# yu45020/Text_Segmentation_Image_Inpainting

Hardware: NVIDIA H100
Metric: PartialConv UNet 512x512 images/sec (fwd+bwd) (higher is better)
Workload: dtype bf16

## Files before the change

text_segmentation_image_inpainting_b200/build.py:

```python
import fcntl
import hashlib
import os
import shutil
import subprocess
import sys

HERE = os.path.dirname(os.path.abspath(__file__))
CSRC = os.path.join(HERE, "csrc")
LIB = os.path.join(HERE, "libpconv_b200.so")
STAMP = os.path.join(HERE, "libpconv_b200.stamp")
SOURCES = ["api.cu", "conv_tc.cu", "conv_smallco.cu", "conv_k2r.cu", "conv_stem.cu", "conv_generic.cu", "elementwise.cu", "dwconv.cu", "seg_ops.cu", "inpaint_data.cu", "inpaint_loss.cu", "seg_data.cu", "seg_loss.cu"]
HEADERS = ["pcb_common.cuh", "pcb_ptx.cuh", "pil_data.cuh", os.path.join("..", "..", "include", "pconv_b200.h")]
NVCC_FLAGS = ["-gencode", "arch=compute_90a,code=sm_90a", "-O3", "-std=c++17", "-lineinfo",
              "-Xcompiler", "-fPIC", "-Xcompiler", "-fvisibility=hidden", "--expt-relaxed-constexpr",
              "-cudart", "static"]


def _nvcc():
    for cand in (os.environ.get("NVCC"), shutil.which("nvcc"), "/usr/local/cuda/bin/nvcc"):
        if cand and os.path.exists(cand):
            return cand
    raise RuntimeError("nvcc not found")


def _fingerprint(sources=None):
    h = hashlib.sha256()
    for d in [os.path.join(CSRC, s) for s in (SOURCES if sources is None else sources) + HEADERS] + [os.path.abspath(__file__)]:
        with open(d, "rb") as f:
            h.update(os.path.basename(d).encode() + b"\0" + f.read() + b"\0")
    h.update(" ".join(NVCC_FLAGS + os.environ.get("PCB_EXTRA_NVCC_FLAGS", "").split()).encode())
    return h.hexdigest()


def needs_build():
    if not os.path.exists(LIB):
        return True
    try:
        with open(STAMP) as f:
            return f.read().strip() != _fingerprint()
    except OSError:
        return True


def build(force=False, verbose=False):
    if not force and not needs_build():
        return LIB
    bdir = os.path.join(HERE, "build")
    os.makedirs(bdir, exist_ok=True)
    with open(os.path.join(bdir, ".lock"), "w") as lockf:
        fcntl.flock(lockf, fcntl.LOCK_EX)
        try:
            if not force and not needs_build():
                return LIB
            return _build_locked(bdir, verbose, force)
        finally:
            fcntl.flock(lockf, fcntl.LOCK_UN)


def _build_locked(bdir, verbose, force=False):
    nvcc = _nvcc()
    fp = _fingerprint()
    tag = f".{os.getpid()}.tmp"
    objs, procs = [], []
    stamps = {}
    for s in SOURCES:
        o = os.path.join(bdir, s.replace(".cu", ".o"))
        objs.append(o)
        stamps[o] = _fingerprint([s])
        try:
            if not force and os.path.exists(o) and open(o + ".stamp").read().strip() == stamps[o]:
                continue
        except OSError:
            pass
        cmd = [nvcc, *NVCC_FLAGS, *os.environ.get("PCB_EXTRA_NVCC_FLAGS", "").split(), "-c", os.path.join(CSRC, s), "-o", o + tag]
        if verbose:
            print(" ".join(cmd))
        procs.append((s, o, subprocess.Popen(cmd, stdout=subprocess.PIPE, stderr=subprocess.STDOUT)))
    failed = None
    for s, _o, p in procs:
        out, _ = p.communicate()
        if p.returncode and failed is None:
            failed = f"nvcc failed on {s}:\n{out.decode()}"
        if verbose and out:
            print(out.decode())
    if failed:
        for _s, o, _p in procs:
            if os.path.exists(o + tag):
                os.remove(o + tag)
        raise RuntimeError(failed)
    for _s, o, _p in procs:
        os.replace(o + tag, o)
        with open(o + ".stamp", "w") as f:
            f.write(stamps[o] + "\n")
    cmd = [nvcc, "-shared", "-o", LIB + tag, *objs, "-cudart", "static"]
    r = subprocess.run(cmd, stdout=subprocess.PIPE, stderr=subprocess.STDOUT)
    if r.returncode:
        raise RuntimeError("link failed:\n" + r.stdout.decode())
    os.replace(LIB + tag, LIB)
    with open(STAMP + tag, "w") as f:
        f.write(fp + "\n")
    os.replace(STAMP + tag, STAMP)
    return LIB


if __name__ == "__main__":
    print(build(force="--force" in sys.argv, verbose=True))
```

text_segmentation_image_inpainting_b200/csrc/conv_stem.cu:

```cuda
#include <string.h>

#include <algorithm>

#include "pcb_common.cuh"

namespace {

constexpr int S2D_C = 32;
constexpr int SK = 4;

size_t rup256(size_t v) { return (v + 255) / 256 * 256; }
size_t s2d_bytes(const pcb_conv *c) { return rup256(static_cast<size_t>(c->n) * (c->h / 2) * (c->w / 2) * S2D_C * sizeof(bf16)); }
size_t dwsub_bytes(const pcb_conv *c) { return rup256(sizeof(float) * c->cout * SK * SK * S2D_C); }

}

StemPlan pcb_stem_plan(const pcb_conv *c) {
    StemPlan K;
    memset(&K, 0, sizeof(K));
    if (c->dtype != PCB_BF16 || c->groups != 1 || c->nparts != 1 || c->kh != 7 || c->kw != 7 || c->stride != 2 || c->pad_h != 3 || c->pad_w != 3 ||
        c->dil != 1) return K;
    const pcb_part &p = c->parts[0];
    if (p.x_up || p.c > 8 || p.x_cstride != 8 || (p.mask && p.mask_up != 0) || ((c->h | c->w) & 1)) return K;
    if (p.x && (reinterpret_cast<uintptr_t>(p.x) & 15)) return K;
    if (c->ho != c->h / 2 || c->wo != c->w / 2 || c->cout < 32 || (c->cout & 7)) return K;
    pcb_conv &S = K.sub;
    S.n = c->n; S.h = c->h / 2; S.w = c->w / 2; S.cin = S2D_C; S.cout = c->cout; S.kh = S.kw = SK; S.stride = 1; S.pad_h = S.pad_w = 2; S.dil = 1;
    S.groups = 1; S.ho = S.h; S.wo = S.w; S.dtype = PCB_BF16; S.no_guard = c->no_guard; S.nparts = 1;
    S.parts[0].x = nullptr; S.parts[0].mask = nullptr; S.parts[0].c = S2D_C; S.parts[0].x_cstride = S2D_C;
    if (!pcb_tc_eligible(&S)) return K;
    size_t de;
    pcb_tc_weight_layout(&S, &K.sub_fe, &de);
    K.sub_fe = (K.sub_fe + 63) / 64 * 64;
    K.fwd_extra = K.sub_fe + 2 * static_cast<size_t>(c->cout) * SK * SK * S2D_C;
    K.workspace = s2d_bytes(c) + dwsub_bytes(c) + pcb_tc_workspace(&S);
    K.ok = true;
    return K;
}

namespace {

__global__ void s2d_kernel(const bf16 *__restrict__ x, const uint8_t *__restrict__ mask, bf16 *__restrict__ xs, int n, int h, int w) {
    const int hs = h >> 1, ws = w >> 1;
    const long long total = static_cast<long long>(n) * hs * ws * 2;
    for (long long i = blockIdx.x * static_cast<long long>(blockDim.x) + threadIdx.x; i < total; i += static_cast<long long>(gridDim.x) * blockDim.x) {
        const int a = static_cast<int>(i & 1);
        const long long cell = i >> 1;
        const int sx = static_cast<int>(cell % ws);
        const long long t = cell / ws;
        const int sy = static_cast<int>(t % hs), img = static_cast<int>(t / hs);
        const long long q = (static_cast<long long>(img) * h + 2 * sy + a) * w + 2 * sx;
        uint4 v0 = __ldg(reinterpret_cast<const uint4 *>(x + q * 8)), v1 = __ldg(reinterpret_cast<const uint4 *>(x + q * 8 + 8));
        if (mask) {
            if (mask[q] == 0) v0 = make_uint4(0u, 0u, 0u, 0u);
            if (mask[q + 1] == 0) v1 = make_uint4(0u, 0u, 0u, 0u);
        }
        uint4 *dst = reinterpret_cast<uint4 *>(xs + cell * S2D_C + a * 16);
        dst[0] = v0; dst[1] = v1;
    }
}

__global__ void stem_weight_kernel(const float *__restrict__ w, float *__restrict__ wsub, int cout, int cin) {
    const int i = blockIdx.x * blockDim.x + threadIdx.x;
    if (i >= cout * SK * SK * S2D_C) return;
    const int k = i % S2D_C, jb = (i / S2D_C) % SK, ja = (i / (S2D_C * SK)) % SK, co = i / (S2D_C * SK * SK);
    const int ch = k & 7, b = (k >> 3) & 1, a = k >> 4;
    const int ty = 2 * ja + a - 1, tx = 2 * jb + b - 1;
    wsub[i] = (ty >= 0 && ty < 7 && tx >= 0 && tx < 7 && ch < cin) ? w[((static_cast<long long>(co) * 7 + ty) * 7 + tx) * cin + ch] : 0.f;
}

__global__ void stem_dw_gather_kernel(const float *__restrict__ dwsub, float *__restrict__ dw, int cout, int cin) {
    const int i = blockIdx.x * blockDim.x + threadIdx.x;
    if (i >= cout * 49 * cin) return;
    const int ch = i % cin, tx = (i / cin) % 7, ty = (i / (cin * 7)) % 7, co = i / (cin * 49);
    const int ja = (ty + 1) >> 1, a = (ty + 1) & 1, jb = (tx + 1) >> 1, b = (tx + 1) & 1;
    dw[i] += dwsub[((static_cast<long long>(co) * SK + ja) * SK + jb) * S2D_C + (a * 2 + b) * 8 + ch];
}

int run_s2d(const pcb_conv *c, bf16 *xs, cudaStream_t st) {
    const pcb_part &p = c->parts[0];
    PCB_CHECK(p.x != nullptr, "space-to-depth stem: null x");
    const long long total = static_cast<long long>(c->n) * (c->h / 2) * (c->w / 2) * 2;
    const int grid = static_cast<int>(std::max<long long>(1, std::min<long long>((total + 255) / 256, 16ll * pcb_num_sms())));
    s2d_kernel<<<grid, 256, 0, st>>>(static_cast<const bf16 *>(p.x), p.mask, xs, c->n, c->h, c->w);
    PCB_LAUNCH_CHECK();
    return 0;
}

}

int pcb_stem_weight_prepare(const pcb_conv *c, const StemPlan &K, const float *w_master, void *w_fwd_extra, bool zero_padding, cudaStream_t st) {
    PCB_CHECK(K.ok && w_fwd_extra, "space-to-depth stem: weight prepare on a layer that does not take this path");
    float *wsub = reinterpret_cast<float *>(static_cast<bf16 *>(w_fwd_extra) + K.sub_fe);
    const int total = c->cout * SK * SK * S2D_C;
    stem_weight_kernel<<<(total + 255) / 256, 256, 0, st>>>(w_master, wsub, c->cout, c->cin);
    PCB_LAUNCH_CHECK();
    return pcb_tc_weight_prepare(&K.sub, wsub, w_fwd_extra, nullptr, zero_padding, st);
}

int pcb_stem_forward(const pcb_conv *c, const StemPlan &K, const void *w_fwd_extra, const float *bias, void *y, int y_cstride,
                     const float *msum, void *workspace, double *bn_sums, const pcb_ep *ep, cudaStream_t st) {
    PCB_CHECK(K.ok && workspace, "space-to-depth stem forward: wrong layer / no workspace");
    uint8_t *ws = static_cast<uint8_t *>(workspace);
    bf16 *xs = reinterpret_cast<bf16 *>(ws);
    if (int rc = run_s2d(c, xs, st)) return rc;
    pcb_conv sub = K.sub;
    sub.parts[0].x = xs;
    uint64_t *sub_ws = reinterpret_cast<uint64_t *>(ws + s2d_bytes(c) + dwsub_bytes(c));
    if (int rc = pcb_tc_forward_mask_pass(&sub, sub_ws, st)) return rc;
    return pcb_tc_forward_ws(&sub, w_fwd_extra, bias, y, y_cstride, msum, sub_ws, true, bn_sums, ep, st);
}

int pcb_stem_wgrad(const pcb_conv *c, const StemPlan &K, const void *dc, int dc_cstride, float *dw, void *workspace, bool zero_dw,
                   cudaStream_t st) {
    PCB_CHECK(K.ok && workspace, "space-to-depth stem wgrad: wrong layer / no workspace");
    if (zero_dw) PCB_CUDA(cudaMemsetAsync(dw, 0, sizeof(float) * c->cout * 49 * c->cin, st));
    uint8_t *ws = static_cast<uint8_t *>(workspace);
    bf16 *xs = reinterpret_cast<bf16 *>(ws);
    float *dwsub = reinterpret_cast<float *>(ws + s2d_bytes(c));
    void *sub_ws = ws + s2d_bytes(c) + dwsub_bytes(c);
    if (int rc = run_s2d(c, xs, st)) return rc;
    pcb_conv sub = K.sub;
    sub.parts[0].x = xs;
    if (int rc = pcb_tc_wgrad(&sub, dc, dc_cstride, dwsub, sub_ws, true, st)) return rc;
    const int total = c->cout * 49 * c->cin;
    stem_dw_gather_kernel<<<(total + 255) / 256, 256, 0, st>>>(dwsub, dw, c->cout, c->cin);
    PCB_LAUNCH_CHECK();
    return 0;
}
```

text_segmentation_image_inpainting_b200/csrc/conv_tc.cu:

```cuda
#include <cuda.h>
#include <stdlib.h>
#include <string.h>

#include <algorithm>

#include "pcb_common.cuh"
#include "pcb_ptx.cuh"

namespace {

constexpr int BLOCK_M = 128;
constexpr int BLOCK_K = 64;
constexpr int A_STAGE_BYTES = BLOCK_M * 128;
constexpr int NUM_PRODUCER_THREADS = 128;
constexpr int TC_MAX_PARTS = 2;
constexpr int MMA_WARPS = 8;
constexpr int MMA_THREADS = MMA_WARPS * 32;
constexpr int acc_pitch(int block_n) { return block_n + 4; }
constexpr int acc_stage_bytes(int block_n) { return BLOCK_M * acc_pitch(block_n) * 4; }

inline int rup(int v, int m) { return (v + m - 1) / m * m; }

struct TcPart {
    const bf16 *x;
    const uint64_t *tapmask;
    const uint8_t *mask;
    bf16 *dx;
    int c, c8, kext, koff, choff, cstride, xup, mup, dx_cstride;
};

struct TcParams {
    int n, h, w, cin, cout, kh, kw, stride, pad_h, pad_w, dil, ho, wo;
    int m_total;
    int nparts, no_guard, rowpack;
    int ncols;
    int ring_a, ring_b;
    int ktap;
    TcPart parts[TC_MAX_PARTS];
    const float *bias; const float *msum; bf16 *y; int y_cstride;
    const bf16 *dc; int dc_cstride, dc_c8, dc_kext;
    const bf16 *relu_x; int relu_cstride;
    int *abort_flag;
    int box_w, box_h, box_n, stages, use_fix;
    int wk_base, wk_row, wk_col;
    int sub, py, px, fh, fw;
    double *bn_sums;
    int bn_c;
    const float *ep_scale, *ep_shift;
    int ep_on, ep_act;
    float ep_slope;
};

constexpr int STAT_SLICE = 256;
constexpr int STAT_SMEM_BYTES = MMA_WARPS * STAT_SLICE * 4 + 16;
constexpr int EPI_WARPS = 4;
constexpr int EPI_STAT_SLICE = 512;
constexpr int EPI_STAT_SQ = EPI_STAT_SLICE / 2;
constexpr int EPI_STAT_SMEM_BYTES = EPI_WARPS * EPI_STAT_SLICE * 4;
constexpr int bf16_pitch(int block_n) { return block_n + 8; }
constexpr int bf16_stage_bytes(int block_n) { return BLOCK_M * bf16_pitch(block_n) * 2; }

__device__ __forceinline__ float warp_transpose_sum16(float (&v)[16], int lane) {
#pragma unroll
    for (int i = 0; i < 16; ++i) v[i] += __shfl_xor_sync(0xffffffffu, v[i], 16);
#pragma unroll
    for (int off = 8, n = 16; off >= 1; off >>= 1, n >>= 1) {
        const bool upper = (lane & off) != 0;
#pragma unroll
        for (int i = 0; i < 8; ++i) {
            if (i < (n >> 1)) {
                const float send = upper ? v[i] : v[i + (n >> 1)];
                const float keep = upper ? v[i + (n >> 1)] : v[i];
                v[i] = keep + __shfl_xor_sync(0xffffffffu, send, off);
            }
        }
    }
    return v[0];
}

__device__ __forceinline__ float warp_transpose_sum(float (&v)[32], int lane) {
#pragma unroll
    for (int off = 16, n = 32; off >= 1; off >>= 1, n >>= 1) {
        const bool upper = (lane & off) != 0;
#pragma unroll
        for (int i = 0; i < 16; ++i) {
            if (i < (n >> 1)) {
                const float send = upper ? v[i] : v[i + (n >> 1)];
                const float keep = upper ? v[i + (n >> 1)] : v[i];
                v[i] = keep + __shfl_xor_sync(0xffffffffu, send, off);
            }
        }
    }
    return v[0];
}

__device__ __forceinline__ uint32_t align1024(uint32_t a) { return (a + 1023u) & ~1023u; }

__device__ __forceinline__ void load_acc32(const float *src, uint32_t (&r)[32]) {
#pragma unroll
    for (int j = 0; j < 8; ++j) {
        const uint4 v = reinterpret_cast<const uint4 *>(src)[j];
        r[4 * j] = v.x; r[4 * j + 1] = v.y; r[4 * j + 2] = v.z; r[4 * j + 3] = v.w;
    }
}

struct EpiRow {
    long long mo;
    int m;
    bool rvalid, hole;
    float inv;
    float dscale[TC_MAX_PARTS];
};

template <int MODE>
__device__ __forceinline__ EpiRow tc_epi_row(const TcParams &P, int m, bool renorm = true) {
    EpiRow er;
    er.m = m;
    er.rvalid = m < P.m_total;
    er.inv = 0.f;
    er.hole = false;
    er.mo = m;
    int en = 0, eh = 0, ew = 0;
    if (MODE == 1 && er.rvalid) {
        en = m / (P.h * P.w); const int rem = m - en * P.h * P.w; eh = rem / P.w; ew = rem - eh * P.w;
        eh = eh * P.sub + P.py; ew = ew * P.sub + P.px;
        er.mo = (static_cast<long long>(en) * P.fh + eh) * P.fw + ew;
    }
    if (MODE == 0 && er.rvalid && renorm) {
        const float s = P.msum ? P.msum[er.mo] : 1.f;
        er.hole = (s == 0.f) && !P.no_guard;
        er.inv = er.hole ? 0.f : 1.0f / s;
    }
#pragma unroll
    for (int p = 0; p < TC_MAX_PARTS; ++p) {
        er.dscale[p] = 1.f;
        if (MODE == 1 && p < P.nparts) {
            const TcPart &pt = P.parts[p];
            if (er.rvalid && pt.dx != nullptr && pt.mask != nullptr)
                er.dscale[p] = pt.mask[(static_cast<long long>(en) * (P.fh >> pt.mup) + (eh >> pt.mup)) * (P.fw >> pt.mup) + (ew >> pt.mup)] ? 1.f : 0.f;
        }
    }
    return er;
}

template <int BLOCK_N, int MODE>
__device__ __forceinline__ void tc_epilogue(const TcParams &P, const EpiRow &er, const float *acc_row, int lane, int n0, float *s_stat,
                                            int cb, int ce, int sq_off) {
                const bool rvalid = er.rvalid, hole = er.hole;
                const long long mo = er.mo;
    #pragma unroll 1
                for (int c0 = cb; c0 < ce; c0 += 32) {
                    uint32_t r[32];
                    load_acc32(acc_row + c0, r);
                    const int col = n0 + c0;
                    bf16 *orow = nullptr;
                    int nstore = 0;
                    float scale = er.inv;
                    if (MODE == 0) {
                        if (rvalid && col < P.y_cstride) { orow = P.y + mo * P.y_cstride + col; nstore = min(32, P.y_cstride - col); }
                    } else {
                        scale = 1.f;
#pragma unroll
                        for (int p = 0; p < TC_MAX_PARTS; ++p) {
                            if (p >= P.nparts) break;
                            const TcPart &pt = P.parts[p];
                            const int local = col - pt.koff;
                            if (local >= 0 && local < pt.kext && pt.dx != nullptr && local < pt.c8 && rvalid) {
                                orow = pt.dx + mo * pt.dx_cstride + local;
                                nstore = min(32, pt.c8 - local);
                                scale = er.dscale[p];
                            }
                        }
                    }
                    const bool stats = (MODE == 0) && (s_stat != nullptr);
                    if (__any_sync(0xffffffffu, nstore > 0) || stats) {
                        uint4 o[4];
                        __nv_bfloat162 *ob = reinterpret_cast<__nv_bfloat162 *>(o);
                        float bl = 0.f;
                        const bool has_bias = (MODE == 0) && (P.bias != nullptr);
                        if (has_bias && col + lane < P.cout) bl = P.bias[col + lane];
                        const bool edge = (MODE == 0) && (col + 32 > P.cout);
                        const bool ep = (MODE == 0) && (P.ep_on != 0);
                        float el = 1.f, eh = 0.f;
                        if (ep && P.ep_scale != nullptr && col + lane < P.cout) { el = P.ep_scale[col + lane]; eh = P.ep_shift[col + lane]; }
    #pragma unroll
                        for (int j = 0; j < 16; ++j) {
                            float a = __uint_as_float(r[2 * j]), b = __uint_as_float(r[2 * j + 1]);
                            if (MODE == 0) {
                                const float b0 = has_bias ? __shfl_sync(0xffffffffu, bl, 2 * j) : 0.f;
                                const float b1 = has_bias ? __shfl_sync(0xffffffffu, bl, 2 * j + 1) : 0.f;
                                a = hole ? 0.f : fmaf(a, scale, b0);
                                b = hole ? 0.f : fmaf(b, scale, b1);
                                if (ep) {
                                    a = apply_act(fmaf(a, __shfl_sync(0xffffffffu, el, 2 * j), __shfl_sync(0xffffffffu, eh, 2 * j)), P.ep_act, P.ep_slope);
                                    b = apply_act(fmaf(b, __shfl_sync(0xffffffffu, el, 2 * j + 1), __shfl_sync(0xffffffffu, eh, 2 * j + 1)), P.ep_act, P.ep_slope);
                                }
                                if (edge) {
                                    if (col + 2 * j >= P.cout) a = 0.f;
                                    if (col + 2 * j + 1 >= P.cout) b = 0.f;
                                }
                            } else {
                                a *= scale; b *= scale;
                            }
                            ob[j] = __floats2bfloat162_rn(a, b);
                        }
                        if (nstore > 0) {
                            uint4 *dst = reinterpret_cast<uint4 *>(orow);
    #pragma unroll
                            for (int j = 0; j < 4; ++j)
                                if (j * 8 < nstore) dst[j] = o[j];
                        }
                        if (stats) {
                            float v[32], q[32];
                            const float live = rvalid ? 1.f : 0.f;
    #pragma unroll
                            for (int j = 0; j < 16; ++j) {
                                const float2 f = __bfloat1622float2(ob[j]);
                                v[2 * j] = f.x * live; v[2 * j + 1] = f.y * live;
                                q[2 * j] = v[2 * j] * v[2 * j]; q[2 * j + 1] = v[2 * j + 1] * v[2 * j + 1];
                            }
                            const float cs = warp_transpose_sum(v, lane), cq = warp_transpose_sum(q, lane);
                            s_stat[c0 - cb + lane] += cs;
                            s_stat[sq_off + c0 - cb + lane] += cq;
                        }
                    }
                }
}

template <int BLOCK_N>
__device__ __forceinline__ void tc_stats_flush(const TcParams &P, float *s_stat, int lane, int n0, int cb, int ce, int sq_off) {
    __syncwarp();
    for (int c0 = cb; c0 < ce; c0 += 32) {
        const int co = n0 + c0 + lane;
        if (co < P.bn_c) {
            atomicAdd(P.bn_sums + co, static_cast<double>(s_stat[c0 - cb + lane]));
            atomicAdd(P.bn_sums + P.bn_c + co, static_cast<double>(s_stat[sq_off + c0 - cb + lane]));
        }
        s_stat[c0 - cb + lane] = 0.f; s_stat[sq_off + c0 - cb + lane] = 0.f;
    }
    __syncwarp();
}

template <int BLOCK_N>
struct EpiRole {
    static constexpr int HN = (BLOCK_N >= 64) ? BLOCK_N / 2 : BLOCK_N;
    int q, half, cb, ce;
    __device__ __forceinline__ explicit EpiRole(int e) {
        q = 2 * (e >> 2) + (e & 1);
        half = (e & 3) >> 1;
        cb = half * HN;
        ce = (cb + HN <= BLOCK_N) ? cb + HN : cb;
    }
    __device__ __forceinline__ int slice() const { return half * 4 + q; }
};

template <int BLOCK_N>
__device__ __forceinline__ void stage_acc(const float (&acc)[BLOCK_N / 2], float *stage, int e, int lane) {
    constexpr int PITCH = acc_pitch(BLOCK_N);
    const int r0 = 64 * (e >> 2) + 16 * (e & 3) + (lane >> 2), c0 = 2 * (lane & 3);
#pragma unroll
    for (int i = 0; i < BLOCK_N / 2; i += 2) {
        const int row = r0 + 8 * ((i >> 1) & 1), col = 8 * (i >> 2) + c0;
        *reinterpret_cast<float2 *>(stage + row * PITCH + col) = make_float2(acc[i], acc[i + 1]);
    }
}

template <int BLOCK_N, int MODE>
__device__ __forceinline__ void mma_epilogue(const TcParams &P, const float (&acc)[BLOCK_N / 2], float *stage, int e, int lane, int m0, int n0,
                                             float *s_stat) {
    constexpr int PITCH = acc_pitch(BLOCK_N);
    const int g = e >> 2;
    stage_acc<BLOCK_N>(acc, stage, e, lane);
    ptx::named_sync(1 + g, 128);
    const EpiRole<BLOCK_N> R(e);
    const EpiRow er = tc_epi_row<MODE>(P, m0 + R.q * 32 + lane);
    tc_epilogue<BLOCK_N, MODE>(P, er, stage + (R.q * 32 + lane) * PITCH, lane, n0, s_stat, R.cb, R.ce, 128);
    ptx::named_sync(1 + g, 128);
}

template <int BLOCK_N>
__device__ __forceinline__ void tc_stats_final(const TcParams &P, const float *stat_base, int w, int lane, int stat_n0) {
    for (int col = w * 32 + lane; col < BLOCK_N; col += EPI_WARPS * 32) {
        const int co = stat_n0 + col;
        if (co < P.bn_c) {
            float a = 0.f, q = 0.f;
#pragma unroll
            for (int w4 = 0; w4 < EPI_WARPS; ++w4) { a += stat_base[w4 * EPI_STAT_SLICE + col]; q += stat_base[w4 * EPI_STAT_SLICE + EPI_STAT_SQ + col]; }
            atomicAdd(P.bn_sums + co, static_cast<double>(a));
            atomicAdd(P.bn_sums + P.bn_c + co, static_cast<double>(q));
        }
    }
}

template <int R> __device__ __forceinline__ void zero_acc(float (&a)[R]) {
#pragma unroll
    for (int i = 0; i < R; ++i) a[i] = 0.f;
}

constexpr int PERSIST_THREADS = 4 * 32 + MMA_THREADS + 32;
constexpr int MAX_RING = 8;

template <int BLOCK_N, int MODE>
__global__ void __launch_bounds__(PERSIST_THREADS, 1)
pconv_tc_persistent_kernel(const __grid_constant__ TcParams P, const __grid_constant__ CUtensorMap tmap_w) {
    constexpr int B_STAGE_BYTES = BLOCK_N * 128;
    extern __shared__ uint8_t smem_raw[];
    const uint32_t smem_base = align1024(ptx::smem_u32(smem_raw));
    const int SA = P.ring_a, SB = P.ring_b;
    const uint32_t sB = smem_base;
    const uint32_t sA = sB + SB * B_STAGE_BYTES;
    const uint32_t sBar = (sA + SA * A_STAGE_BYTES + 15u) & ~15u;
    const uint32_t bar_full_a = sBar, bar_empty_a = sBar + 8 * MAX_RING;
    const uint32_t bar_full_b = sBar + 16 * MAX_RING, bar_empty_b = sBar + 24 * MAX_RING;
    const uint32_t s_stat_addr = sBar + 32 * MAX_RING;
    const uint32_t s_acc = (s_stat_addr + STAT_SMEM_BYTES + 15u) & ~15u;
    float *acc_stage = reinterpret_cast<float *>(smem_raw + (s_acc - ptx::smem_u32(smem_raw)));

    const int warp = threadIdx.x >> 5, lane = threadIdx.x & 31;
    const int taps = P.kh * P.kw;
    const int np = (MODE == 0) ? P.nparts : 1;
    const int n_tiles = P.ncols / BLOCK_N;
    const int num_tiles = ((P.m_total + BLOCK_M - 1) / BLOCK_M) * n_tiles;

    auto tile_active = [&](int n0) -> bool {
        if (MODE == 0) return true;
        for (int p = 0; p < P.nparts; ++p)
            if (P.parts[p].dx && n0 < P.parts[p].koff + P.parts[p].kext && n0 + BLOCK_N > P.parts[p].koff) return true;
        return false;
    };

    if (threadIdx.x == 0) {
        for (int s = 0; s < MAX_RING; ++s) {
            ptx::mbar_init(bar_full_a + 8 * s, NUM_PRODUCER_THREADS); ptx::mbar_init(bar_empty_a + 8 * s, 2);
            ptx::mbar_init(bar_full_b + 8 * s, 1); ptx::mbar_init(bar_empty_b + 8 * s, 2);
        }
        ptx::fence_mbar_init();
    }
    if (warp == 12 && lane == 0) ptx::prefetch_tmap(&tmap_w);
    __syncthreads();

    if (warp < 4) {
        const int t = threadIdx.x;
        const int chunk = t & 7, r0 = t >> 3;
        const int plane = (MODE == 0) ? P.ho * P.wo : P.h * P.w;
        const int pwid = (MODE == 0) ? P.wo : P.w;
        int it = 0;
        bool dead = false;
        uint64_t wnext[TC_MAX_PARTS][8];
        auto issue_mask_loads = [&](int tl) {
#pragma unroll
            for (int p = 0; p < TC_MAX_PARTS; ++p)
#pragma unroll
                for (int i = 0; i < 8; ++i) wnext[p][i] = 0ull;
            if (MODE != 0 || tl >= num_tiles) return;
            const int tm0 = (tl / n_tiles) * BLOCK_M;
#pragma unroll
            for (int i = 0; i < 8; ++i) {
                const int idx = tm0 + r0 + 16 * i;
                if (idx >= P.m_total) continue;
#pragma unroll
                for (int p = 0; p < TC_MAX_PARTS; ++p)
                    if (p < P.nparts) wnext[p][i] = __ldg(P.parts[p].tapmask + idx);
            }
        };
        issue_mask_loads(blockIdx.x);
        for (int tile = blockIdx.x; tile < num_tiles && !dead; tile += gridDim.x) {
            const int m0 = (tile / n_tiles) * BLOCK_M, n0 = (tile % n_tiles) * BLOCK_N;
            uint64_t wcur[TC_MAX_PARTS][8];
#pragma unroll
            for (int p = 0; p < TC_MAX_PARTS; ++p)
#pragma unroll
                for (int i = 0; i < 8; ++i) wcur[p][i] = wnext[p][i];
            issue_mask_loads(tile + gridDim.x);
            if (!tile_active(n0)) continue;
            const uint32_t sw = static_cast<uint32_t>((chunk ^ (r0 & 7)) << 4);
            int ph[8], pw[8];
            int ibase[TC_MAX_PARTS][8];
            bool prow[8];
            const int ls = 31 - __clz(P.stride);
#pragma unroll
            for (int i = 0; i < 8; ++i) {
                const int m = m0 + r0 + 16 * i;
                prow[i] = m < P.m_total;
                const int mm = prow[i] ? m : 0;
                const int nn = mm / plane, rem = mm - nn * plane;
                const int hh = rem / pwid, ww = rem - hh * pwid;
                if (MODE == 0) {
                    ph[i] = hh * P.stride - P.pad_h; pw[i] = ww * P.stride - P.pad_w;
#pragma unroll
                    for (int p = 0; p < TC_MAX_PARTS; ++p)
                        ibase[p][i] = (p < P.nparts) ? nn * (P.h >> P.parts[p].xup) * (P.w >> P.parts[p].xup) * P.parts[p].cstride + chunk * 8 : 0;
                } else {
                    ph[i] = hh + P.pad_h; pw[i] = ww + P.pad_w;
                    ibase[0][i] = nn * P.ho * P.wo * P.dc_cstride + chunk * 8;
#pragma unroll
                    for (int p = 1; p < TC_MAX_PARTS; ++p) ibase[p][i] = 0;
                }
            }
            uint64_t tmv[TC_MAX_PARTS][8];
#pragma unroll
            for (int p = 0; p < TC_MAX_PARTS; ++p)
#pragma unroll
                for (int i = 0; i < 8; ++i) tmv[p][i] = wcur[p][i];

            auto push = [&](const bf16 *base, const int (&off)[8], const bool (&ok)[8]) -> bool {
                const int s = it % SA;
                if (!ptx::mbar_wait(bar_empty_a + 8 * s, ((it / SA) & 1) ^ 1, P.abort_flag, 101)) return false;
                const uint32_t dst = sA + s * A_STAGE_BYTES + r0 * 128 + sw;
#pragma unroll
                for (int i = 0; i < 8; ++i) ptx::cp_async_16(dst + i * (16 * 128), base + off[i], ok[i]);
                ptx::cp_async_mbar_arrive(bar_full_a + 8 * s);
                ptx::mbar_arrive(bar_full_a + 8 * s);
                ++it;
                return true;
            };
            if (MODE == 0 && P.rowpack) {
                const TcPart &pt = P.parts[0];
                const int cs = pt.cstride, rowpitch = P.w * cs;
                for (int tr = 0; tr < P.kh && !dead; ++tr) {
                    int off[8];
                    bool ok[8];
#pragma unroll
                    for (int i = 0; i < 8; ++i) {
                        const bool v = (chunk < P.kw) && ((tmv[0][i] >> (tr * P.kw + chunk)) & 1ull);
                        off[i] = v ? (ibase[0][i] - chunk * 8) + (ph[i] + tr * P.dil) * rowpitch + (pw[i] + chunk * P.dil) * cs : 0;
                        ok[i] = v;
                    }
                    if (!push(pt.x, off, ok)) dead = true;
                }
            } else {
                for (int tap = 0; tap < taps && !dead; ++tap) {
                    const int tr = tap / P.kw, tc = tap - tr * P.kw;
#pragma unroll
                    for (int p = 0; p < TC_MAX_PARTS; ++p) {
                        if (p >= np || dead) break;
                        const TcPart &pt = P.parts[p];
                        const bf16 *src = (MODE == 0) ? pt.x : P.dc;
                        const int cs = (MODE == 0) ? pt.cstride : P.dc_cstride;
                        const int xup = (MODE == 0) ? pt.xup : 0;
                        const int rowpitch = ((MODE == 0) ? (P.w >> xup) : P.wo) * cs;
                        int base[8];
                        bool rv[8];
#pragma unroll
                        for (int i = 0; i < 8; ++i) {
                            bool v;
                            int hi, wi;
                            if (MODE == 0) {
                                v = (tmv[p][i] >> tap) & 1ull;
                                hi = (ph[i] + tr * P.dil) >> xup; wi = (pw[i] + tc * P.dil) >> xup;
                            } else {
                                const int th = ph[i] - tr * P.dil, tw = pw[i] - tc * P.dil;
                                hi = th >> ls; wi = tw >> ls;
                                v = prow[i] && th >= 0 && tw >= 0 && ((th | tw) & (P.stride - 1)) == 0 && hi < P.ho && wi < P.wo;
                            }
                            base[i] = v ? ibase[p][i] + hi * rowpitch + wi * cs : 0;
                            rv[i] = v;
                        }
                        const int nb = ((MODE == 0) ? pt.kext : P.dc_kext) / BLOCK_K;
                        const int c8 = (MODE == 0) ? pt.c8 : P.dc_c8;
                        for (int cb = 0; cb < nb; ++cb) {
                            const bool cv = cb * BLOCK_K + chunk * 8 < c8;
                            int off[8];
                            bool ok[8];
#pragma unroll
                            for (int i = 0; i < 8; ++i) { ok[i] = rv[i] && cv; off[i] = ok[i] ? base[i] + cb * BLOCK_K : 0; }
                            if (!push(src, off, ok)) { dead = true; break; }
                        }
                    }
                }
            }
        }
        ptx::cp_async_wait<0>();
    } else if (warp == 12) {
        if (lane == 0) {
            int itb = 0;
            bool dead = false;
            auto load = [&](int kidx, int n0) -> bool {
                const int s = itb % SB;
                if (!ptx::mbar_wait(bar_empty_b + 8 * s, ((itb / SB) & 1) ^ 1, P.abort_flag, 103)) return false;
                ptx::mbar_arrive_expect_tx(bar_full_b + 8 * s, B_STAGE_BYTES);
                ptx::tma_load_2d(sB + s * B_STAGE_BYTES, &tmap_w, kidx, n0, bar_full_b + 8 * s);
                ++itb;
                return true;
            };
            for (int tile = blockIdx.x; tile < num_tiles && !dead; tile += gridDim.x) {
                const int n0 = (tile % n_tiles) * BLOCK_N;
                if (!tile_active(n0)) continue;
                const int num_kb = (MODE == 0) ? (P.rowpack ? P.kh : taps * (P.ktap / BLOCK_K)) : taps * (P.dc_kext / BLOCK_K);
                for (int kb = 0; kb < num_kb; ++kb)
                    if (!load(kb * BLOCK_K, n0)) { dead = true; break; }
            }
        }
    } else {
        const int e = warp - 4, g = e >> 2;
        const bool leader = (threadIdx.x & 127) == 0;
        const int num_a = (MODE == 0) ? (P.rowpack ? P.kh : taps * (P.ktap / BLOCK_K)) : taps * (P.dc_kext / BLOCK_K);
        const uint32_t a_rows = 64u * 128u;
        float *s_stat = (MODE == 0 && P.bn_sums != nullptr)
                            ? reinterpret_cast<float *>(smem_raw + (s_stat_addr - ptx::smem_u32(smem_raw))) : nullptr;
        const EpiRole<BLOCK_N> R(e);
        float *my_stat = s_stat ? s_stat + R.slice() * STAT_SLICE : nullptr;
        int stat_n0 = -1;
        if (my_stat) {
            for (int i = lane; i < STAT_SLICE; i += 32) my_stat[i] = 0.f;
            __syncwarp();
        }
        int ita = 0, itb = 0;
        bool dead = false;
        for (int tile = blockIdx.x; tile < num_tiles && !dead; tile += gridDim.x) {
            const int m0 = (tile / n_tiles) * BLOCK_M, n0 = (tile % n_tiles) * BLOCK_N;
            if (!tile_active(n0)) continue;
            if (my_stat && n0 != stat_n0) {
                if (stat_n0 >= 0) tc_stats_flush<BLOCK_N>(P, my_stat, lane, stat_n0, R.cb, R.ce, 128);
                stat_n0 = n0;
            }
            float acc[BLOCK_N / 2];
            zero_acc(acc);
            for (int a = 0; a < num_a && !dead; ++a, ++ita) {
                const int sa = ita % SA;
                if (!__all_sync(0xffffffffu, ptx::mbar_wait(bar_full_a + 8 * sa, (ita / SA) & 1, P.abort_flag, 104))) { dead = true; break; }
                ptx::fence_proxy_async_smem();
                const int sb = itb % SB;
                if (__all_sync(0xffffffffu, ptx::mbar_wait(bar_full_b + 8 * sb, (itb / SB) & 1, P.abort_flag, 105))) {
                    const uint64_t db = ptx::make_smem_desc(sB + sb * B_STAGE_BYTES, 16, 1024);
                    ptx::wgmma_fence();
                    const uint64_t da = ptx::make_smem_desc(sA + sa * A_STAGE_BYTES + g * a_rows, 16, 1024);
#pragma unroll
                    for (int k = 0; k < BLOCK_K / 16; ++k)
                        ptx::wgmma_bf16<BLOCK_N, 0, 0>(acc, da + 2 * k, db + 2 * k);
                    ptx::wgmma_commit();
                    ++itb;
                } else {
                    dead = true;
                }
                ptx::wgmma_wait<0>();
                ptx::wgmma_fence_regs(acc);
                if (leader) {
                    ptx::mbar_arrive(bar_empty_b + 8 * sb);
                    ptx::mbar_arrive(bar_empty_a + 8 * sa);
                }
            }
            if (dead) { stat_n0 = -1; break; }
            mma_epilogue<BLOCK_N, MODE>(P, acc, acc_stage, e, lane, m0, n0, my_stat);
        }
        if (my_stat && stat_n0 >= 0) tc_stats_flush<BLOCK_N>(P, my_stat, lane, stat_n0, R.cb, R.ce, 128);
    }
}


constexpr int EPI_WARP0 = MMA_WARPS + 4;
constexpr int TMA_THREADS = (EPI_WARP0 + EPI_WARPS) * 32;
constexpr int TMA_FIX_THREADS = 96;
constexpr int TMA_REGS = 128;
constexpr int TMA_CONSUMER_REGS = 192, TMA_SUPPORT_REGS = 64;
static_assert(TMA_THREADS == 512 && 2 * 128 * TMA_CONSUMER_REGS + 2 * 128 * TMA_SUPPORT_REGS == TMA_THREADS * TMA_REGS &&
              TMA_THREADS * TMA_REGS <= 65536, "TMA-fed fwd / dgrad register budget");

constexpr size_t TMA_BAR_BYTES = 24 * MAX_RING + 16;

template <int BLOCK_N, int MODE>
__device__ __forceinline__ void tc_epilogue_bf16(const TcParams &P, const EpiRow &er, const bf16 *srow, int lane, int n0, float *s_stat) {
    const bool stats = (MODE == 0) && (s_stat != nullptr);
#pragma unroll 1
    for (int c0 = 0; c0 < BLOCK_N; c0 += 32) {
        const int col = n0 + c0;
        bf16 *orow = nullptr;
        int nstore = 0;
        int xlocal = 0;
        float scale = 1.f;
        if (MODE == 0) {
            if (er.rvalid && col < P.y_cstride) { orow = P.y + er.mo * P.y_cstride + col; nstore = min(32, P.y_cstride - col); }
        } else {
#pragma unroll
            for (int p = 0; p < TC_MAX_PARTS; ++p) {
                if (p >= P.nparts) break;
                const TcPart &pt = P.parts[p];
                const int local = col - pt.koff;
                if (local >= 0 && local < pt.kext && pt.dx != nullptr && local < pt.c8 && er.rvalid) {
                    orow = pt.dx + er.mo * pt.dx_cstride + local;
                    nstore = min(32, pt.c8 - local);
                    scale = er.dscale[p];
                    xlocal = local;
                }
            }
        }
        if (nstore == 0 && !stats) continue;
        uint4 o[4];
#pragma unroll
        for (int j = 0; j < 4; ++j) o[j] = reinterpret_cast<const uint4 *>(srow + c0)[j];
        if (MODE == 1 && scale != 1.f) {
            __nv_bfloat162 *ob = reinterpret_cast<__nv_bfloat162 *>(o);
#pragma unroll
            for (int j = 0; j < 16; ++j) {
                const float2 f = __bfloat1622float2(ob[j]);
                ob[j] = __floats2bfloat162_rn(f.x * scale, f.y * scale);
            }
        }
        if (MODE == 1 && P.relu_x != nullptr && nstore > 0) {
            const uint4 *xr = reinterpret_cast<const uint4 *>(P.relu_x + er.mo * P.relu_cstride + xlocal);
#pragma unroll 1
            for (int j = 0; j < 4; ++j) {
                if (j * 8 >= nstore) break;
                const uint4 xv = xr[j];
                const __nv_bfloat162 *xb = reinterpret_cast<const __nv_bfloat162 *>(&xv);
                __nv_bfloat162 *ob = reinterpret_cast<__nv_bfloat162 *>(&o[j]);
#pragma unroll
                for (int k = 0; k < 4; ++k) {
                    const float2 xf = __bfloat1622float2(xb[k]);
                    const __nv_bfloat162 z = __float2bfloat162_rn(0.f);
                    ob[k] = __halves2bfloat162(xf.x <= 0.f ? z.x : ob[k].x, xf.y <= 0.f ? z.y : ob[k].y);
                }
            }
        }
        if (nstore > 0) {
            uint4 *dst = reinterpret_cast<uint4 *>(orow);
#pragma unroll
            for (int j = 0; j < 4; ++j)
                if (j * 8 < nstore) dst[j] = o[j];
        }
        if (stats) {
            const float live = er.rvalid ? 1.f : 0.f;
            const __nv_bfloat162 *ob = reinterpret_cast<const __nv_bfloat162 *>(srow + c0);
            float cs = 0.f, cq = 0.f;
#pragma unroll 1
            for (int h = 0; h < 2; ++h) {
                float v[16];
#pragma unroll
                for (int j = 0; j < 8; ++j) {
                    const float2 f = __bfloat1622float2(ob[8 * h + j]);
                    v[2 * j] = f.x * live; v[2 * j + 1] = f.y * live;
                }
                const float s = warp_transpose_sum16(v, lane);
#pragma unroll
                for (int j = 0; j < 8; ++j) {
                    const float2 f = __bfloat1622float2(ob[8 * h + j]);
                    const float a = f.x * live, b = f.y * live;
                    v[2 * j] = a * a; v[2 * j + 1] = b * b;
                }
                const float q = warp_transpose_sum16(v, lane);
                if ((lane >> 4) == h) { cs = s; cq = q; }
            }
            s_stat[c0 + lane] += cs;
            s_stat[EPI_STAT_SQ + c0 + lane] += cq;
        }
    }
}

template <int BLOCK_N, int MODE, typename TileFn>
__device__ __forceinline__ void tma_epilogue_warps(const TcParams &P, int tile0, int tstep, int num_tiles, TileFn tile_origin,
                                                   const bf16 *stage, uint32_t acc_full, uint32_t acc_empty, float *s_stat,
                                                   int &stat_n0, int w, int lane, int code) {
    const int row = w * 32 + lane;
    if (s_stat) {
        for (int i = lane; i < EPI_STAT_SLICE; i += 32) s_stat[i] = 0.f;
        __syncwarp();
    }
    uint32_t ph = 0;
    for (int tile = tile0; tile < num_tiles; tile += tstep) {
        int m0, n0;
        tile_origin(tile, m0, n0);
        if (n0 < 0) continue;
        if (s_stat && n0 != stat_n0) {
            if (stat_n0 >= 0) tc_stats_flush<BLOCK_N>(P, s_stat, lane, stat_n0, 0, BLOCK_N, EPI_STAT_SQ);
            stat_n0 = n0;
        }
        const EpiRow er = tc_epi_row<MODE>(P, m0 + row, false);
        if (!__all_sync(0xffffffffu, ptx::mbar_wait(acc_full, ph, P.abort_flag, code))) { stat_n0 = -1; return; }
        ph ^= 1;
        tc_epilogue_bf16<BLOCK_N, MODE>(P, er, stage + row * bf16_pitch(BLOCK_N), lane, n0, s_stat);
        __syncwarp();
        if (lane == 0) ptx::mbar_arrive(acc_empty);
    }
}

struct ConsRows {
    float inv[2];
    bool hole[2];
};
template <int MODE>
__device__ __forceinline__ ConsRows cons_rows(const TcParams &P, int m0, int e, int lane) {
    ConsRows cr;
#pragma unroll
    for (int h = 0; h < 2; ++h) {
        cr.inv[h] = 0.f; cr.hole[h] = false;
        if (MODE == 0) {
            const EpiRow er = tc_epi_row<0>(P, m0 + 64 * (e >> 2) + 16 * (e & 3) + (lane >> 2) + 8 * h);
            cr.inv[h] = er.inv; cr.hole[h] = er.hole;
        }
    }
    return cr;
}

template <int BLOCK_N, int MODE>
__device__ __forceinline__ void stage_acc_bf16(const TcParams &P, const float (&acc)[BLOCK_N / 2], bf16 *stage, int e, int lane, int n0,
                                               const ConsRows &cr) {
    constexpr int PITCH = bf16_pitch(BLOCK_N);
    const int r0 = 64 * (e >> 2) + 16 * (e & 3) + (lane >> 2), c0 = 2 * (lane & 3);
    const bool has_bias = (MODE == 0) && (P.bias != nullptr);
    const bool ep = (MODE == 0) && (P.ep_on != 0);
    const bool ep_aff = ep && (P.ep_scale != nullptr);
#pragma unroll
    for (int j = 0; j < BLOCK_N / 8; ++j) {
        const int col = n0 + 8 * j + c0;
        float b0 = 0.f, b1 = 0.f, s0 = 1.f, s1 = 1.f, t0 = 0.f, t1 = 0.f;
        if (MODE == 0) {
            const bool in0 = col < P.cout, in1 = col + 1 < P.cout;
            if (has_bias) { if (in0) b0 = __ldg(P.bias + col); if (in1) b1 = __ldg(P.bias + col + 1); }
            if (ep_aff) {
                if (in0) { s0 = __ldg(P.ep_scale + col); t0 = __ldg(P.ep_shift + col); }
                if (in1) { s1 = __ldg(P.ep_scale + col + 1); t1 = __ldg(P.ep_shift + col + 1); }
            }
        }
#pragma unroll
        for (int h = 0; h < 2; ++h) {
            float a = acc[4 * j + 2 * h], b = acc[4 * j + 2 * h + 1];
            if (MODE == 0) {
                a = cr.hole[h] ? 0.f : fmaf(a, cr.inv[h], b0);
                b = cr.hole[h] ? 0.f : fmaf(b, cr.inv[h], b1);
                if (ep) {
                    a = apply_act(fmaf(a, s0, t0), P.ep_act, P.ep_slope);
                    b = apply_act(fmaf(b, s1, t1), P.ep_act, P.ep_slope);
                }
                if (col >= P.cout) a = 0.f;
                if (col + 1 >= P.cout) b = 0.f;
            }
            *reinterpret_cast<__nv_bfloat162 *>(stage + (r0 + 8 * h) * PITCH + 8 * j + c0) = __floats2bfloat162_rn(a, b);
        }
    }
}

template <int BLOCK_N, int MODE>
__device__ __forceinline__ bool tma_stage_tile(const TcParams &P, const float (&acc)[BLOCK_N / 2], bf16 *stage, uint32_t acc_full,
                                               uint32_t acc_empty, uint32_t &ph, int e, int lane, int n0, const ConsRows &cr, int code) {
    if (!__all_sync(0xffffffffu, ptx::mbar_wait(acc_empty, ph, P.abort_flag, code))) return false;
    ph ^= 1;
    stage_acc_bf16<BLOCK_N, MODE>(P, acc, stage, e, lane, n0, cr);
    __syncwarp();
    if (lane == 0) ptx::mbar_arrive(acc_full);
    return true;
}

template <int BLOCK_N, int MODE, bool HALO>
__global__ void __maxnreg__(TMA_REGS)
pconv_tc_tma_kernel(const __grid_constant__ TcParams P, const __grid_constant__ CUtensorMap tmap_w,
                    const __grid_constant__ CUtensorMap tmap_a0, const __grid_constant__ CUtensorMap tmap_a1) {
    constexpr uint32_t B_BYTES = BLOCK_N * 128;
    extern __shared__ uint8_t smem_raw[];
    const uint32_t smem_base = align1024(ptx::smem_u32(smem_raw));
    const int S = P.stages;
    const int nB = HALO ? P.kw : 1;
    const int hx = HALO ? (P.kw - 1) * P.dil : 0;
    const uint32_t A_BYTES = static_cast<uint32_t>(BLOCK_M + hx) * 128u;
    const uint32_t A_ROOM = (A_BYTES + 1023u) & ~1023u;
    const uint32_t STAGE = A_ROOM + nB * B_BYTES;
    const uint32_t STAGE_TX = A_BYTES + nB * B_BYTES;
    const uint32_t sBar = smem_base + S * STAGE;
    const uint32_t bar_full = sBar, bar_fixed = sBar + 8 * MAX_RING, bar_empty = sBar + 16 * MAX_RING;
    const uint32_t acc_full = sBar + 24 * MAX_RING, acc_empty = acc_full + 8;
    const uint32_t s_stat_addr = sBar + TMA_BAR_BYTES;
    const uint32_t s_acc = s_stat_addr + EPI_STAT_SMEM_BYTES;
    uint8_t *smem_gen = smem_raw + (smem_base - ptx::smem_u32(smem_raw));

    const int warp = __shfl_sync(0xffffffffu, threadIdx.x >> 5, 0), lane = threadIdx.x & 31;
    const int np = (MODE == 0) ? P.nparts : 1;
    const int n_tiles = P.ncols / BLOCK_N;
    const int m_tiles = (P.m_total + BLOCK_M - 1) / BLOCK_M;
    const int num_tiles = m_tiles * n_tiles;
    const int tile0 = static_cast<int>(blockIdx.x), tstep = static_cast<int>(gridDim.x);
    auto m0_of = [&](int mt) -> int { return mt * BLOCK_M; };
    const bool fix = (MODE == 0) && P.use_fix;
    const int kwi = HALO ? 1 : P.kw;

    auto tile_active = [&](int n0) -> bool {
        if (MODE == 0) return true;
        for (int p = 0; p < P.nparts; ++p)
            if (P.parts[p].dx && n0 < P.parts[p].koff + P.parts[p].kext && n0 + BLOCK_N > P.parts[p].koff) return true;
        return false;
    };

    if (threadIdx.x == 0) {
        for (int s = 0; s < MAX_RING; ++s) {
            ptx::mbar_init(bar_full + 8 * s, 1); ptx::mbar_init(bar_fixed + 8 * s, TMA_FIX_THREADS / 32); ptx::mbar_init(bar_empty + 8 * s, 2);
        }
        ptx::mbar_init(acc_full, MMA_WARPS); ptx::mbar_init(acc_empty, EPI_WARPS);
        ptx::fence_mbar_init();
    }
    if (warp == 8 && lane == 0) { ptx::prefetch_tmap(&tmap_w); ptx::prefetch_tmap(&tmap_a0); if (np > 1) ptx::prefetch_tmap(&tmap_a1); }
    __syncthreads();

    float *s_stat = nullptr;
    int stat_n0 = -1;
    bf16 *acc_stage = reinterpret_cast<bf16 *>(smem_gen + (s_acc - smem_base));
    if (warp < MMA_WARPS) {
        ptx::setmaxnreg_inc<TMA_CONSUMER_REGS>();
        const int e = warp, g = warp >> 2;
        const bool leader = (threadIdx.x & 127) == 0;
        const uint32_t ready = fix ? bar_fixed : bar_full;
        const uint64_t desc_a0 = ptx::make_smem_desc(smem_base + g * 64 * 128, 16, 1024);
        const uint64_t desc_b0 = ptx::make_smem_desc(smem_base + A_ROOM, 16, 1024);
        const uint32_t stage16 = STAGE >> 4;
        const int shift0 = (HALO && MODE == 1) ? hx * 8 : 0;
        const int dshift = HALO ? ((MODE == 1) ? -P.dil * 8 : P.dil * 8) : 0;
        const int rows_a = P.kh * kwi;
        int nb0, nb1 = 0, kl0, kl1 = 4;
        {
            const int kext = (MODE == 0) ? P.parts[0].kext : P.dc_kext, c8 = (MODE == 0) ? P.parts[0].c8 : P.dc_c8;
            nb0 = kext / BLOCK_K; kl0 = min(4, (c8 - (nb0 - 1) * BLOCK_K + 15) >> 4);
            if (MODE == 0 && np > 1) { nb1 = P.parts[1].kext / BLOCK_K; kl1 = min(4, (P.parts[1].c8 - (nb1 - 1) * BLOCK_K + 15) >> 4); }
        }
        int s = 0;
        uint32_t ph = 0, aph = 1;
        bool dead = false;
        for (int tile = tile0; tile < num_tiles && !dead; tile += tstep) {
            const int n0 = (tile % n_tiles) * BLOCK_N;
            if (!tile_active(n0)) continue;
            const ConsRows cr = cons_rows<MODE>(P, m0_of(tile / n_tiles), e, lane);
            float acc[BLOCK_N / 2];
            zero_acc(acc);
            int held = -1;
            for (int r = 0; r < rows_a && !dead; ++r) {
#pragma unroll
                for (int p = 0; p < TC_MAX_PARTS; ++p) {
                    const int nbp = (p == 0) ? nb0 : nb1, klast = (p == 0) ? kl0 : kl1;
                    for (int cb = 0; cb < nbp; ++cb) {
                        if (!__all_sync(0xffffffffu, ptx::mbar_wait(ready + 8 * s, ph, P.abort_flag, 124))) { dead = true; break; }
                        uint64_t da = desc_a0 + static_cast<uint64_t>(s * stage16 + shift0), db = desc_b0 + static_cast<uint64_t>(s * stage16);
                        const int ksteps = (cb + 1 < nbp) ? 4 : klast;
                        ptx::wgmma_fence();
                        for (int tc = 0; tc < nB; ++tc, da += dshift, db += B_BYTES >> 4) {
                            if (ksteps == 4) {
#pragma unroll
                                for (int k = 0; k < 4; ++k) ptx::wgmma_bf16<BLOCK_N, 0, 0>(acc, da + 2 * k, db + 2 * k);
                            } else {
                                for (int k = 0; k < ksteps; ++k) ptx::wgmma_bf16<BLOCK_N, 0, 0>(acc, da + 2 * k, db + 2 * k);
                            }
                        }
                        ptx::wgmma_commit();
                        ptx::wgmma_wait<1>();
                        if (held >= 0 && leader) ptx::mbar_arrive(bar_empty + 8 * held);
                        held = s;
                        if (++s == S) { s = 0; ph ^= 1; }
                    }
                    if (dead) break;
                }
            }
            ptx::wgmma_wait<0>();
            ptx::wgmma_fence_regs(acc);
            if (held >= 0 && leader) ptx::mbar_arrive(bar_empty + 8 * held);
            if (dead) break;
            if (!tma_stage_tile<BLOCK_N, MODE>(P, acc, acc_stage, acc_full, acc_empty, aph, e, lane, n0, cr, 125)) break;
        }
    } else {
        ptx::setmaxnreg_dec<TMA_SUPPORT_REGS>();
        if (warp >= EPI_WARP0) {
            const int w = warp - EPI_WARP0;
            s_stat = (MODE == 0 && P.bn_sums != nullptr)
                         ? reinterpret_cast<float *>(smem_gen + (s_stat_addr - smem_base)) + w * EPI_STAT_SLICE : nullptr;
            auto origin = [&](int tile, int &m0, int &n0) {
                m0 = m0_of(tile / n_tiles); n0 = (tile % n_tiles) * BLOCK_N;
                if (!tile_active(n0)) n0 = -1;
            };
            tma_epilogue_warps<BLOCK_N, MODE>(P, tile0, tstep, num_tiles, origin, acc_stage, acc_full, acc_empty, s_stat, stat_n0, w, lane, 126);
            ptx::named_sync(1, EPI_WARPS * 32);
            if (s_stat != nullptr && stat_n0 >= 0) tc_stats_final<BLOCK_N>(P, s_stat - w * EPI_STAT_SLICE, w, lane, stat_n0);
        } else if (warp == 8) {
            int s = 0;
            uint32_t ph = 1;
            const int plane = (MODE == 0) ? P.ho * P.wo : P.h * P.w;
            const int pwid = (MODE == 0) ? P.wo : P.w;
            const int kext0 = (MODE == 0) ? P.parts[0].kext : P.dc_kext, kext1 = (MODE == 0 && np > 1) ? P.parts[1].kext : 0;
            const int dstep = (MODE == 0) ? P.dil : -P.dil;
            const int row_k = P.wk_row, col_k = P.wk_col;
            bool dead = false;
            for (int tile = tile0; tile < num_tiles && !dead; tile += tstep) {
                const int m0 = m0_of(tile / n_tiles), n0 = (tile % n_tiles) * BLOCK_N;
                if (!tile_active(n0)) continue;
                const int img = m0 / plane, rem = m0 - img * plane;
                const int oy = rem / pwid, ox = rem - oy * pwid;
                const int x_org = (MODE == 0) ? ox * P.stride - P.pad_w : (HALO ? ox + P.pad_w - hx : ox + P.pad_w);
                const int y_org = (MODE == 0) ? oy * P.stride - P.pad_h : oy + P.pad_h;
                int krow = P.wk_base;
                for (int tr = 0, y = y_org; tr < P.kh && !dead; ++tr, y += dstep, krow += row_k)
                    for (int ti = 0, x = x_org, kidx = krow; ti < kwi && !dead; ++ti, x += dstep, kidx = krow + ti * col_k) {
#pragma unroll
                        for (int p = 0; p < TC_MAX_PARTS; ++p) {
                            const int kext = (p == 0) ? kext0 : kext1;
                            const CUtensorMap *ma = (p == 0) ? &tmap_a0 : &tmap_a1;
                            for (int c0 = 0; c0 < kext; c0 += BLOCK_K, kidx += BLOCK_K) {
                                if (!__all_sync(0xffffffffu, ptx::mbar_wait(bar_empty + 8 * s, ph, P.abort_flag, 121))) { dead = true; break; }
                                if (ptx::elect_one()) {
                                    const uint32_t full = bar_full + 8 * s, dst = smem_base + s * STAGE;
                                    ptx::mbar_arrive_expect_tx(full, STAGE_TX);
                                    ptx::tma_load_4d(dst, ma, c0, x, y, img, full);
                                    uint32_t bdst = dst + A_ROOM;
                                    for (int tc = 0, kb = kidx; tc < nB; ++tc, kb += col_k, bdst += B_BYTES)
                                        ptx::tma_load_2d(bdst, &tmap_w, kb, n0, full);
                                }
                                __syncwarp();
                                if (++s == S) { s = 0; ph ^= 1; }
                            }
                            if (dead) break;
                        }
                    }
            }
        } else {
            if (fix) {
                constexpr int FR = HALO ? 3 : 2;
                const int t = (warp - 9) * 32 + lane;
                int s = 0;
                uint32_t ph = 0;
                bool dead = false;
                auto zero_row = [&](int row) {
                    uint4 *r = reinterpret_cast<uint4 *>(smem_gen + s * STAGE + row * 128);
                    const uint4 z = make_uint4(0u, 0u, 0u, 0u);
#pragma unroll
                    for (int k = 0; k < 8; ++k) r[k] = z;
                };
                if (!HALO) {
                    uint64_t wnext[FR][TC_MAX_PARTS];
                    auto load_words = [&](int tl) {
#pragma unroll
                        for (int r = 0; r < FR; ++r)
#pragma unroll
                            for (int p = 0; p < TC_MAX_PARTS; ++p) {
                                wnext[r][p] = 0ull;
                                const int m = m0_of(tl / n_tiles) + t + TMA_FIX_THREADS * r;
                                if (p < P.nparts && tl < num_tiles && t + TMA_FIX_THREADS * r < BLOCK_M && m < P.m_total)
                                    wnext[r][p] = __ldg(P.parts[p].tapmask + m);
                            }
                    };
                    load_words(tile0);
                    for (int tile = tile0; tile < num_tiles && !dead; tile += tstep) {
                        uint64_t wcur[FR][TC_MAX_PARTS];
#pragma unroll
                        for (int r = 0; r < FR; ++r)
#pragma unroll
                            for (int p = 0; p < TC_MAX_PARTS; ++p) wcur[r][p] = wnext[r][p];
                        load_words(tile + tstep);
                        if (MODE == 1 && !tile_active((tile % n_tiles) * BLOCK_N)) continue;
                        const int taps = P.kh * P.kw;
                        for (int tap = 0; tap < taps && !dead; ++tap) {
#pragma unroll
                            for (int p = 0; p < TC_MAX_PARTS; ++p) {
                                if (p >= np) break;
                                bool hole[FR], mine = false;
#pragma unroll
                                for (int r = 0; r < FR; ++r) {
                                    hole[r] = t + TMA_FIX_THREADS * r < BLOCK_M && ((wcur[r][p] >> tap) & 1ull) == 0ull;
                                    mine = mine || hole[r];
                                }
                                const bool any_hole = __any_sync(0xffffffffu, mine);
                                const int nb = ((MODE == 0) ? P.parts[p].kext : P.dc_kext) / BLOCK_K;
                                for (int cb = 0; cb < nb; ++cb) {
                                    if (!ptx::mbar_wait(bar_full + 8 * s, ph, P.abort_flag, 122)) { dead = true; break; }
                                    if (any_hole) {
#pragma unroll
                                        for (int r = 0; r < FR; ++r)
                                            if (hole[r]) zero_row(t + TMA_FIX_THREADS * r);
                                        ptx::fence_proxy_async_smem();
                                    }
                                    __syncwarp();
                                    if (lane == 0) ptx::mbar_arrive(bar_fixed + 8 * s);
                                    if (++s == S) { s = 0; ph ^= 1; }
                                }
                                if (dead) break;
                            }
                        }
                    }
                } else {
                    const int plane = P.ho * P.wo;
                    auto load_bits = [&](int tl, uint32_t (&b)[FR]) {
#pragma unroll
                        for (int r = 0; r < FR; ++r) b[r] = 0;
                        if (tl >= num_tiles) return;
                        const int m0 = m0_of(tl / n_tiles);
                        const int img = m0 / plane, rem = m0 - img * plane;
                        const int oy = rem / P.wo, ox = rem - oy * P.wo;
#pragma unroll
                        for (int p = 0; p < TC_MAX_PARTS; ++p) {
                            if (p >= P.nparts || P.parts[p].mask == nullptr) continue;
                            const int mup = P.parts[p].mup;
                            const uint8_t *mk = P.parts[p].mask + static_cast<long long>(img) * (P.h >> mup) * (P.w >> mup);
                            for (int tr = 0; tr < P.kh; ++tr) {
                                const int y = oy - P.pad_h + tr * P.dil;
                                if (y < 0 || y >= P.h) continue;
#pragma unroll
                                for (int r = 0; r < FR; ++r) {
                                    const int row = t + TMA_FIX_THREADS * r, x = ox - P.pad_w + row;
                                    if (row < BLOCK_M + hx && x >= 0 && x < P.w && __ldg(mk + (y >> mup) * (P.w >> mup) + (x >> mup)) == 0)
                                        b[r] |= 1u << (p * 8 + tr);
                                }
                            }
                        }
                    };
                    uint32_t nb_bits[FR];
                    load_bits(tile0, nb_bits);
                    for (int tile = tile0; tile < num_tiles && !dead; tile += tstep) {
                        uint32_t cb_bits[FR];
#pragma unroll
                        for (int r = 0; r < FR; ++r) cb_bits[r] = nb_bits[r];
                        load_bits(tile + tstep, nb_bits);
                        if (MODE == 1 && !tile_active((tile % n_tiles) * BLOCK_N)) continue;
                        for (int tr = 0; tr < P.kh && !dead; ++tr) {
#pragma unroll
                            for (int p = 0; p < TC_MAX_PARTS; ++p) {
                                if (p >= np) break;
                                bool hole[FR], mine = false;
#pragma unroll
                                for (int r = 0; r < FR; ++r) { hole[r] = (cb_bits[r] >> (p * 8 + tr)) & 1u; mine = mine || hole[r]; }
                                const bool any_hole = __any_sync(0xffffffffu, mine);
                                const int nb = ((MODE == 0) ? P.parts[p].kext : P.dc_kext) / BLOCK_K;
                                for (int cb = 0; cb < nb; ++cb) {
                                    if (!ptx::mbar_wait(bar_full + 8 * s, ph, P.abort_flag, 122)) { dead = true; break; }
                                    if (any_hole) {
#pragma unroll
                                        for (int r = 0; r < FR; ++r)
                                            if (hole[r]) zero_row(t + TMA_FIX_THREADS * r);
                                        ptx::fence_proxy_async_smem();
                                    }
                                    __syncwarp();
                                    if (lane == 0) ptx::mbar_arrive(bar_fixed + 8 * s);
                                    if (++s == S) { s = 0; ph ^= 1; }
                                }
                                if (dead) break;
                            }
                        }
                    }
                }
            }
        }
    }

}


constexpr int SP_MAX_ITEMS = 40;
struct SpItem { int dx, dy, wk; };
struct SpTable {
    int n_items;
    SpItem it[SP_MAX_ITEMS];
};

template <int BLOCK_N>
// ... 1264 lines not shown
    memset(ta, 0, sizeof(ta));
    for (int p = 0; p < c->nparts; ++p) {
        const pcb_part &pt = c->parts[p];
        const void *src = pt.x;
        long long cs = pt.x_cstride;
        const int c8 = rup(pt.c, 8);
        if (pt.x_up) {
            bf16 *up = reinterpret_cast<bf16 *>(static_cast<uint8_t *>(workspace) + T.up_off[p]);
            const long long pix = static_cast<long long>(c->n) * (c->h >> 1) * (c->w >> 1);
            const long long work = pix * (c8 >> 3);
            const int grid = static_cast<int>(std::min<long long>((work + 255) / 256, 16ll * pcb_num_sms()));
            upsample_part_kernel<<<grid, 256, 0, st>>>(static_cast<const bf16 *>(pt.x), pt.x_cstride, c8, pix, c->h >> 1, c->w >> 1, up);
            PCB_LAUNCH_CHECK();
            src = up; cs = c8;
        }
        if (pt.mask) *use_fix = 1;
        if (int rc = make_tmap_nhwc(&ta[p], src, c8, c->w, c->h, c->n, cs, bx, by, bn, c->stride)) return rc;
    }
    if (c->nparts < 2) ta[1] = ta[0];
    return 0;
}

pcb_smallco_layout smallco_layout(const Layout &L) {
    pcb_smallco_layout S;
    S.ktap = L.ktap; S.koff[0] = L.koff[0]; S.koff[1] = L.koff[1]; S.cout64 = L.cout64; S.kf = L.kf; S.kd = L.kd;
    return S;
}

}

bool pcb_tc_eligible(const pcb_conv *c) { return common_ok(c); }

size_t pcb_tc_workspace(const pcb_conv *c) { return tc_plan(c).workspace; }

void pcb_tc_weight_layout(const pcb_conv *c, size_t *fwd_elems, size_t *dgrad_elems) {
    const TcPlan T = tc_plan(c);
    *fwd_elems = T.fwd_elems;
    *dgrad_elems = T.dg_elems;
}

bool pcb_tc_subpixel(const pcb_conv *c) { return tc_plan(c).dg_at_source; }

void pcb_tc_routes(const pcb_conv *c, int32_t routes[3]) {
    static const int32_t code[] = {PCB_ROUTE_NONE, PCB_ROUTE_STEM, PCB_ROUTE_K2R, PCB_ROUTE_SMALLCO, PCB_ROUTE_TMA, PCB_ROUTE_TMA_S2,
                                   PCB_ROUTE_GATHER};
    const TcPlan T = tc_plan(c);
    routes[0] = code[T.fwd.route]; routes[1] = code[T.dg.route]; routes[2] = code[T.wg.route];
}

int pcb_tc_weight_prepare(const pcb_conv *c, const float *w_master, void *w_fwd, void *w_dgrad, bool zero_padding, cudaStream_t st) {
    const TcPlan T = tc_plan(c);
    const Layout &L = T.L;
    const size_t fe = T.fwd_elems, de = T.dg_elems;
    if (zero_padding) {
        PCB_CUDA(cudaMemsetAsync(w_fwd, 0, fe * 2, st));
        if (w_dgrad && de) PCB_CUDA(cudaMemsetAsync(w_dgrad, 0, de * 2, st));
    }
    WPrepParams W;
    memset(&W, 0, sizeof(W));
    W.cout = c->cout; W.taps = c->kh * c->kw; W.cin = c->cin; W.kw = c->kw; W.rowpack = L.rowpack; W.nparts = c->nparts;
    W.ktap = L.ktap; W.cout64 = L.cout64; W.kf = L.kf; W.kd = L.kd;
    int off = 0;
    for (int p = 0; p < c->nparts; ++p) { W.choff[p] = off; W.c[p] = c->parts[p].c; W.koff[p] = L.koff[p]; off += c->parts[p].c; }
    bf16 *wf = static_cast<bf16 *>(w_fwd), *wd = static_cast<bf16 *>(w_dgrad);
    if (!L.rowpack && W.taps <= 65535 && c->cout >= 32 && c->cin >= 32) {
        dim3 tg((c->cin + 31) / 32, (c->cout + 31) / 32, W.taps);
        tc_weight_prepare_tiled_kernel<<<tg, 256, 0, st>>>(w_master, W, wf, (w_dgrad && de) ? wd : nullptr);
    } else {
        const long long total = static_cast<long long>(c->cout) * W.taps * c->cin;
        const int grid = static_cast<int>(std::min<long long>((total + 1023) / 1024, 8ll * pcb_num_sms()));
        tc_weight_prepare_kernel<<<grid < 1 ? 1 : grid, 256, 0, st>>>(w_master, W, wf, (w_dgrad && de) ? wd : nullptr);
    }
    PCB_LAUNCH_CHECK();
    if (T.fwd.route == ROUTE_STEM) return pcb_stem_weight_prepare(c, T.stem, w_master, wf + T.extra_fwd_off, zero_padding, st);
    if (T.fwd.route == ROUTE_K2R) {
        PCB_CHECK(w_dgrad != nullptr, "kernel-to-row weights need the dgrad operand buffer");
        return pcb_k2r_weight_prepare(c, T.k2r, w_master, wf + T.extra_fwd_off, wd + T.extra_dg_off, zero_padding, st);
    }
    if (T.sp.ok) {
        PCB_CHECK(w_dgrad != nullptr, "sub-pixel weights need the dgrad operand buffer");
        return sp_weight_prepare(c, T.sp, L, w_master, wd + T.sp_off, st);
    }
    return 0;
}

int pcb_tc_forward_mask_pass(const pcb_conv *c, uint64_t *tapmask, cudaStream_t st) {
    const TcPlan T = tc_plan(c);
    PCB_CHECK(T.m_out < (1ll << 31), "problem too large");
    return T.fwd_tapmask ? launch_tapmask(c, tapmask, st) : 0;
}

bool pcb_tc_fuses_epilogue(const pcb_conv *c) { return tc_plan(c).fuses_epilogue; }

int pcb_tc_forward_ws(const pcb_conv *c, const void *w_fwd, const float *bias, void *y, int y_cstride, const float *msum,
                      uint64_t *tapmask, bool mask_pass_done, double *bn_sums, const pcb_ep *ep, cudaStream_t st) {
    int *flag = abort_flag_ptr();
    PCB_CHECK(flag != nullptr, "cudaMalloc(abort flag) failed");
    const TcPlan T = tc_plan(c);
    const Layout &L = T.L;
    const DirPlan &F = T.fwd;
    PCB_CHECK(T.m_out < (1ll << 31), "problem too large");
    PCB_CHECK(y_cstride % 8 == 0 && y_cstride >= c->cout, "tensor-core forward: y channel stride must be a multiple of 8 and >= cout");
    PCB_CHECK(bn_sums == nullptr || T.fuses_epilogue, "fused BatchNorm statistics requested from a kernel that does not produce them");
    PCB_CHECK(ep == nullptr || T.fuses_epilogue, "fused BatchNorm + activation requested from a kernel that does not apply it");
    if (!mask_pass_done && T.fwd_tapmask)
        if (int rc = launch_tapmask(c, tapmask, st)) return rc;
    const bf16 *wf = static_cast<const bf16 *>(w_fwd);
    if (F.route == ROUTE_STEM) return pcb_stem_forward(c, T.stem, wf + T.extra_fwd_off, bias, y, y_cstride, msum, tapmask, bn_sums, ep, st);
    if (F.route == ROUTE_K2R) return pcb_k2r_forward(c, T.k2r, smallco_layout(L), w_fwd, wf + T.extra_fwd_off, bias, y, y_cstride, msum, tapmask, st);
    if (F.route == ROUTE_SMALLCO) return pcb_smallco_forward(c, smallco_layout(L), w_fwd, bias, y, y_cstride, msum, st);
    TcParams P;
    base_params(P, c, L);
    P.m_total = static_cast<int>(T.m_out);
    fill_parts(c, L, P.parts, tapmask, T.m_out);
    P.bias = bias; P.msum = msum; P.y = static_cast<bf16 *>(y); P.y_cstride = y_cstride; P.abort_flag = flag;
    P.bn_sums = bn_sums; P.bn_c = c->cout;
    set_ep(P, ep);
    P.ncols = L.rows_f;
    CUtensorMap tm;
    if (int rc = make_tmap_2d(&tm, w_fwd, L.rows_f, L.kf, L.kf, F.bn)) return rc;
    if (F.route == ROUTE_TMA) {
        P.box_w = F.box_w; P.box_h = F.box_h; P.box_n = F.box_n;
        CUtensorMap ta[TC_MAX_PARTS];
        if (int rc = a_operand_maps(c, T, tapmask, F.box_w + (F.halo ? (c->kw - 1) * c->dil : 0), F.box_h, F.box_n, ta, &P.use_fix, st)) return rc;
        P.ncols = (c->cout <= 32) ? 32 : L.rows_f;
        P.wk_base = 0; P.wk_col = L.ktap; P.wk_row = c->kw * L.ktap;
        return launch_tma<0>(P, tm, ta[0], ta[1], F.bn, F.halo, st);
    }
    return launch_tc<0>(P, tm, F.bn, st);
}

bool pcb_tc_dgrad_fuses_relu(const pcb_conv *c) { return tc_plan(c).dg_fuses_relu; }

int pcb_tc_dgrad(const pcb_conv *c, const void *dc, int dc_cstride, const void *w_dgrad, void *const *dx, const int *dx_cstride,
                 cudaStream_t st, const void *relu_x, int relu_cstride) {
    const TcPlan T = tc_plan(c);
    const Layout &L = T.L;
    const DirPlan &D = T.dg;
    PCB_CHECK(D.route != ROUTE_NONE, "data gradient of a row-packed (cin <= 8) tensor-core layer: set force_generic and pass KRSC weights");
    PCB_CHECK(w_dgrad != nullptr && (reinterpret_cast<uintptr_t>(dc) & 15) == 0, "pcb_pconv_backward_data: w_dgrad required / dc misaligned");
    PCB_CHECK(relu_x == nullptr || (T.dg_fuses_relu && relu_cstride % 8 == 0 && relu_cstride >= rup(c->cin, 8) &&
                                    (reinterpret_cast<uintptr_t>(relu_x) & 15) == 0),
              "tensor-core dgrad: the ReLU backward is fused only on the TMA-fed stride-1 kernel (16-byte aligned input, channel stride %% 8 == 0)");
    int *flag = abort_flag_ptr();
    PCB_CHECK(flag != nullptr, "cudaMalloc(abort flag) failed");
    PCB_CHECK(T.m_in < (1ll << 31), "problem too large");
    PCB_CHECK(dc_cstride % 8 == 0 && dc_cstride >= rup(c->cout, 8), "tensor-core dgrad: dc channel stride must be a multiple of 8");
    const bf16 *wd = static_cast<const bf16 *>(w_dgrad);
    if (D.route == ROUTE_K2R) return pcb_k2r_dgrad(c, T.k2r, smallco_layout(L), dc, dc_cstride, w_dgrad, wd + T.extra_dg_off, dx, dx_cstride, st);
    if (D.route == ROUTE_SMALLCO) return pcb_smallco_dgrad(c, smallco_layout(L), dc, dc_cstride, w_dgrad, dx, dx_cstride, st);
    const SpPlan &SPL = T.sp;
    void *dx_local[TC_MAX_PARTS] = {nullptr, nullptr};
    for (int p = 0; p < c->nparts && p < TC_MAX_PARTS; ++p) dx_local[p] = dx[p];
    if (SPL.ok) {
        if (dx[SPL.pu] != nullptr)
            if (int rc = sp_dgrad_up(c, SPL, L, dc, dc_cstride, wd + T.sp_off, dx[SPL.pu], dx_cstride[SPL.pu], flag, st)) return rc;
        dx_local[SPL.pu] = nullptr;
        if (SPL.ps < 0 || dx[SPL.ps] == nullptr) return 0;
    }
    dx = dx_local;
    TcParams P;
    base_params(P, c, L);
    P.m_total = static_cast<int>(T.m_in);
    fill_parts(c, L, P.parts, nullptr, 0);
    for (int p = 0; p < c->nparts; ++p) {
        P.parts[p].dx = static_cast<bf16 *>(dx[p]);
        P.parts[p].dx_cstride = dx_cstride[p];
        PCB_CHECK(!dx[p] || (dx_cstride[p] % 8 == 0 && dx_cstride[p] >= P.parts[p].c8 && (reinterpret_cast<uintptr_t>(dx[p]) & 15) == 0),
                  "tensor-core dgrad: dx[%d] must be 16-byte aligned with a channel stride that is a multiple of 8", p);
    }
    P.dc = static_cast<const bf16 *>(dc); P.dc_cstride = dc_cstride; P.dc_c8 = rup(c->cout, 8); P.dc_kext = L.cout64;
    P.relu_x = static_cast<const bf16 *>(relu_x); P.relu_cstride = relu_cstride;
    P.abort_flag = flag;
    P.ncols = L.ktap;
    CUtensorMap tm;
    if (int rc = make_tmap_2d(&tm, w_dgrad, rup(L.ktap, 128), L.kd, L.kd, D.bn)) return rc;
    if (D.route == ROUTE_TMA) {
        P.box_w = D.box_w; P.box_h = D.box_h; P.box_n = D.box_n;
        P.wk_base = 0; P.wk_col = L.cout64; P.wk_row = c->kw * L.cout64;
        CUtensorMap ta;
        if (int rc = make_tmap_nhwc(&ta, dc, P.dc_c8, c->wo, c->ho, c->n, dc_cstride, D.box_w + (D.halo ? (c->kw - 1) * c->dil : 0), D.box_h, D.box_n, 1)) return rc;
        return launch_tma<1>(P, tm, ta, ta, D.bn, D.halo, st);
    }
    if (D.route == ROUTE_TMA_S2) {
        const int hh = c->h / 2, hw = c->w / 2;
        P.box_w = D.box_w; P.box_h = D.box_h; P.box_n = D.box_n;
        const bool fork = T.cls_fork;
        ClassStreams *CS = nullptr;
        if (fork) {
            if (int rc = class_streams(&CS)) return rc;
            PCB_CUDA(cudaEventRecord(CS->ev_fork, st));
        }
        for (int cls = 0; cls < 4; ++cls) {
            TcParams Q = P;
            const int py = cls >> 1, px = cls & 1;
            const int tr0 = (py + c->pad_h) & 1, tc0 = (px + c->pad_w) & 1;
            Q.kh = (c->kh - tr0 + 1) / 2; Q.kw = class_kw(c, px);
            Q.pad_h = (py + c->pad_h - tr0) / 2; Q.pad_w = (px + c->pad_w - tc0) / 2;
            Q.h = hh; Q.w = hw; Q.stride = 1; Q.dil = 1;
            Q.m_total = static_cast<int>(static_cast<long long>(c->n) * hh * hw);
            Q.sub = 2; Q.py = py; Q.px = px; Q.fh = c->h; Q.fw = c->w;
            Q.wk_base = (tr0 * c->kw + tc0) * L.cout64; Q.wk_row = 2 * c->kw * L.cout64; Q.wk_col = 2 * L.cout64;
            const bool halo = T.cls_halo[cls];
            CUtensorMap ta;
            if (int rc = make_tmap_nhwc(&ta, dc, P.dc_c8, c->wo, c->ho, c->n, dc_cstride, Q.box_w + (halo ? Q.kw - 1 : 0), Q.box_h, Q.box_n, 1)) return rc;
            cudaStream_t cs = (fork && cls > 0) ? CS->aux[cls - 1] : st;
            if (fork && cls > 0) PCB_CUDA(cudaStreamWaitEvent(cs, CS->ev_fork, 0));
            if (int rc = launch_tma<1>(Q, tm, ta, ta, D.bn, halo, cs)) return rc;
            if (fork && cls > 0) {
                PCB_CUDA(cudaEventRecord(CS->ev_join[cls - 1], cs));
                PCB_CUDA(cudaStreamWaitEvent(st, CS->ev_join[cls - 1], 0));
            }
        }
        return 0;
    }
    return launch_tc<1>(P, tm, D.bn, st);
}


template <int BLOCK_N, int T, bool HALO>
int launch_wgrad_tma(WgParams &P, const CUtensorMap &tdc, const CUtensorMap &ta0, const CUtensorMap &ta1, cudaStream_t st) {
    const int rows_a = 64 + (HALO ? (P.kw - 1) * P.dil : 0);
    PCB_CHECK(rows_a <= (HALO ? 3 : 1) * WGRAD_FIX_THREADS, "TMA-fed wgrad: %d-row A blocks exceed the fixer warps", rows_a);
    const size_t a_blk = (static_cast<size_t>(rows_a) * 128 + 1023) / 1024 * 1024;
    const size_t stage = (HALO ? 1 : T) * 2 * a_blk + static_cast<size_t>(BLOCK_N) * 128;
    P.stages = static_cast<int>(std::min<size_t>(MAX_RING, RING_BUDGET / stage));
    PCB_CHECK(P.stages >= 2, "TMA-fed wgrad: stage of %zu bytes does not fit twice", stage);
    const size_t smem = 1024 + P.stages * stage + 24 * MAX_RING;
    auto kern = pconv_tc_wgrad_tma_kernel<BLOCK_N, T, HALO>;
    PCB_SMEM_OPT_IN(kern, MAX_SMEM);
    P.tap_groups = HALO ? P.kh : (P.kh * P.kw + T - 1) / T;
    P.ci_tiles = (P.ktap + 127) / 128;
    const int co_tiles = (P.cout + BLOCK_N - 1) / BLOCK_N;
    const int base_ctas = co_tiles * P.tap_groups * P.ci_tiles;
    const int total_kb = (P.m_total + 63) / 64;
    int splits = (2 * pcb_num_sms() + base_ctas - 1) / base_ctas;
    splits = std::max(1, std::min(splits, total_kb));
    splits = std::min(splits, 65535);
    P.kb_per_split = (total_kb + splits - 1) / splits;
    splits = (total_kb + P.kb_per_split - 1) / P.kb_per_split;
    dim3 grid(base_ctas, splits);
    kern<<<grid, WGRAD_TMA_THREADS, smem, st>>>(P, tdc, ta0, ta1);
    PCB_LAUNCH_CHECK();
    return 0;
}

template <int BLOCK_N, int T, int STAGES>
static int launch_wgrad(WgParams &P, const CUtensorMap &tm, int cout, cudaStream_t st) {
    constexpr size_t smem = 1024 + STAGES * (T * 16384 + BLOCK_N * 128) + 24 * STAGES;
    auto kern = pconv_tc_wgrad_kernel<BLOCK_N, T, STAGES>;
    PCB_SMEM_OPT_IN(kern, (int)smem);
    P.tap_groups = (P.ntaps + T - 1) / T;
    P.ci_tiles = (P.ktap + 127) / 128;
    const int co_tiles = (cout + BLOCK_N - 1) / BLOCK_N;
    const int base_ctas = co_tiles * P.tap_groups * P.ci_tiles;
    const int total_kb = (P.m_total + 63) / 64;
    int splits = (4 * pcb_num_sms() + base_ctas - 1) / base_ctas;
    splits = std::max(1, std::min(splits, total_kb));
    splits = std::min(splits, 65535);
    P.kb_per_split = (total_kb + splits - 1) / splits;
    splits = (total_kb + P.kb_per_split - 1) / P.kb_per_split;
    dim3 grid(base_ctas, splits);
    kern<<<grid, WGRAD_THREADS, smem, st>>>(P, tm);
    PCB_LAUNCH_CHECK();
    return 0;
}

int pcb_tc_wgrad(const pcb_conv *c, const void *dc, int dc_cstride, float *dw, void *workspace, bool zero_dw, cudaStream_t st) {
    int *flag = abort_flag_ptr();
    PCB_CHECK(flag != nullptr, "cudaMalloc(abort flag) failed");
    PCB_CHECK(workspace != nullptr, "pcb_tc_wgrad: workspace required");
    const TcPlan T = tc_plan(c);
    const Layout &L = T.L;
    const DirPlan &W = T.wg;
    PCB_CHECK(T.m_out < (1ll << 31), "problem too large");
    PCB_CHECK(dc_cstride % 8 == 0 && dc_cstride >= c->cout, "tensor-core wgrad: dc channel stride must be a multiple of 8");
    if (W.route == ROUTE_STEM) return pcb_stem_wgrad(c, T.stem, dc, dc_cstride, dw, workspace, zero_dw, st);
    if (W.route == ROUTE_K2R) return pcb_k2r_wgrad(c, T.k2r, dc, dc_cstride, dw, workspace, zero_dw, st);
    if (W.route == ROUTE_SMALLCO) return pcb_smallco_wgrad(c, smallco_layout(L), dc, dc_cstride, dw, zero_dw, st);
    uint64_t *tapmask = static_cast<uint64_t *>(workspace);
    if (T.wg_tapmask)
        if (int rc = launch_tapmask(c, tapmask, st)) return rc;
    const size_t dw_bytes = sizeof(float) * c->cout * c->kh * c->kw * c->cin;
    if (zero_dw) PCB_CUDA(cudaMemsetAsync(dw, 0, dw_bytes, st));
    WgParams P;
    memset(&P, 0, sizeof(P));
    P.n = c->n; P.h = c->h; P.w = c->w; P.cin = c->cin; P.cout = c->cout; P.kh = c->kh; P.kw = c->kw; P.stride = c->stride;
    P.pad_h = c->pad_h; P.pad_w = c->pad_w; P.dil = c->dil; P.ho = c->ho; P.wo = c->wo; P.m_total = static_cast<int>(T.m_out);
    P.nparts = c->nparts; P.rowpack = L.rowpack; P.ktap = L.ktap; P.ntaps = L.rowpack ? c->kh : c->kh * c->kw;
    fill_parts(c, L, P.parts, tapmask, T.m_out);
    P.dw = dw; P.abort_flag = flag;
    CUtensorMap tm;
    if (int rc = make_tmap_2d(&tm, dc, T.m_out, c->cout, dc_cstride, 64)) return rc;
    if (W.route == ROUTE_TMA) {
        P.box_w = W.box_w; P.box_h = W.box_h; P.box_n = W.box_n;
        CUtensorMap ta[TC_MAX_PARTS];
        if (int rc = a_operand_maps(c, T, workspace, W.box_w + (W.halo ? (c->kw - 1) * c->dil : 0), W.box_h, W.box_n, ta, &P.use_fix, st)) return rc;
        if (W.bn == 128) return W.halo ? launch_wgrad_tma<128, 3, true>(P, tm, ta[0], ta[1], st) : launch_wgrad_tma<128, 3, false>(P, tm, ta[0], ta[1], st);
        return W.halo ? launch_wgrad_tma<64, 3, true>(P, tm, ta[0], ta[1], st) : launch_wgrad_tma<64, 3, false>(P, tm, ta[0], ta[1], st);
    }
    return launch_wgrad<64, 3, 3>(P, tm, c->cout, st);
}

int pcb_tc_read_abort_flag(int *value) {
    int *flag = abort_flag_ptr();
    PCB_CHECK(flag != nullptr, "no abort flag");
    PCB_CUDA(cudaMemcpy(value, flag, sizeof(int), cudaMemcpyDeviceToHost));
    if (*value != 0) cudaMemset(flag, 0, sizeof(int));
    return 0;
}
```

text_segmentation_image_inpainting_b200/csrc/pcb_common.cuh:

```cuda
#pragma once
#include <cuda_bf16.h>
#include <cuda_runtime.h>
#include <stdint.h>
#include <stdio.h>

#include "../../include/pconv_b200.h"

int pcb_set_error(const char *fmt, ...);
void pcb_count_launch(int n = 1);

#define PCB_CHECK(cond, ...)                       \
    do {                                           \
        if (!(cond)) return pcb_set_error(__VA_ARGS__); \
    } while (0)

#define PCB_CUDA(expr)                                                                           \
    do {                                                                                         \
        cudaError_t _e = (expr);                                                                 \
        if (_e != cudaSuccess)                                                                   \
            return pcb_set_error("%s:%d: %s -> %s", __FILE__, __LINE__, #expr, cudaGetErrorString(_e)); \
    } while (0)

#define PCB_LAUNCH_CHECK()                                                                        \
    do {                                                                                         \
        cudaError_t _e = cudaGetLastError();                                                     \
        if (_e != cudaSuccess)                                                                   \
            return pcb_set_error("%s:%d: kernel launch -> %s", __FILE__, __LINE__, cudaGetErrorString(_e)); \
        pcb_count_launch();                                                                      \
    } while (0)

constexpr int PCB_MAX_DEVICES = 64;

static inline int pcb_cur_device() {
    int dev = 0;
    cudaGetDevice(&dev);
    return (dev >= 0 && dev < PCB_MAX_DEVICES) ? dev : 0;
}

static inline int pcb_num_sms() {
    static int sms[PCB_MAX_DEVICES] = {0};
    const int dev = pcb_cur_device();
    if (!sms[dev]) {
        int v = 0;
        cudaDeviceGetAttribute(&v, cudaDevAttrMultiProcessorCount, dev);
        sms[dev] = v > 0 ? v : 132;
    }
    return sms[dev];
}

#define PCB_SMEM_OPT_IN(kern, bytes)                                                                          \
    do {                                                                                                      \
        static bool pcb_done_[PCB_MAX_DEVICES] = {};                                                          \
        const int pcb_dev_ = pcb_cur_device();                                                                \
        if (!pcb_done_[pcb_dev_]) {                                                                           \
            PCB_CUDA(cudaFuncSetAttribute(kern, cudaFuncAttributeMaxDynamicSharedMemorySize, (int)(bytes))); \
            pcb_done_[pcb_dev_] = true;                                                                       \
        }                                                                                                     \
    } while (0)

static inline size_t pcb_dtype_size(int dtype) { return dtype == PCB_BF16 ? 2 : 4; }

typedef __nv_bfloat16 bf16;

template <typename T> __device__ __forceinline__ float to_f32(T v);
template <> __device__ __forceinline__ float to_f32<float>(float v) { return v; }
template <> __device__ __forceinline__ float to_f32<bf16>(bf16 v) { return __bfloat162float(v); }

template <typename T> __device__ __forceinline__ T from_f32(float v);
template <> __device__ __forceinline__ float from_f32<float>(float v) { return v; }
template <> __device__ __forceinline__ bf16 from_f32<bf16>(float v) { return __float2bfloat16_rn(v); }

constexpr float PCB_SIGMOID_HALF_THRESHOLD = 8.940696716308594e-08f;
__device__ __forceinline__ bool sigmoid_above_half(float x) { return x > PCB_SIGMOID_HALF_THRESHOLD; }

__device__ __forceinline__ float apply_act(float z, int act, float slope) {
    if (act == PCB_ACT_RELU) return z > 0.f ? z : 0.f;
    if (act == PCB_ACT_LEAKY) return z > 0.f ? z : z * slope;
    if (act == PCB_ACT_RELU6) return fminf(fmaxf(z, 0.f), 6.f);
    return z;
}
__device__ __forceinline__ float act_grad(float z, int act, float slope) {
    if (act == PCB_ACT_RELU) return z > 0.f ? 1.f : 0.f;
    if (act == PCB_ACT_LEAKY) return z > 0.f ? 1.f : slope;
    if (act == PCB_ACT_RELU6) return (z > 0.f && z < 6.f) ? 1.f : 0.f;
    return 1.f;
}

template <typename T> struct Vec8;
template <> struct Vec8<bf16> {
    static __device__ __forceinline__ void load(const bf16 *p, float (&v)[8]) {
        uint4 r = *reinterpret_cast<const uint4 *>(p);
        const __nv_bfloat162 *h = reinterpret_cast<const __nv_bfloat162 *>(&r);
#pragma unroll
        for (int i = 0; i < 4; ++i) {
            float2 f = __bfloat1622float2(h[i]);
            v[2 * i] = f.x;
            v[2 * i + 1] = f.y;
        }
    }
    static __device__ __forceinline__ void store(bf16 *p, const float (&v)[8]) {
        uint4 r;
        __nv_bfloat162 *h = reinterpret_cast<__nv_bfloat162 *>(&r);
#pragma unroll
        for (int i = 0; i < 4; ++i) h[i] = __floats2bfloat162_rn(v[2 * i], v[2 * i + 1]);
        *reinterpret_cast<uint4 *>(p) = r;
    }
};
template <> struct Vec8<float> {
    static __device__ __forceinline__ void load(const float *p, float (&v)[8]) {
        float4 a = reinterpret_cast<const float4 *>(p)[0], b = reinterpret_cast<const float4 *>(p)[1];
        v[0] = a.x; v[1] = a.y; v[2] = a.z; v[3] = a.w; v[4] = b.x; v[5] = b.y; v[6] = b.z; v[7] = b.w;
    }
    static __device__ __forceinline__ void store(float *p, const float (&v)[8]) {
        reinterpret_cast<float4 *>(p)[0] = make_float4(v[0], v[1], v[2], v[3]);
        reinterpret_cast<float4 *>(p)[1] = make_float4(v[4], v[5], v[6], v[7]);
    }
};

__device__ __forceinline__ float warp_sum(float v) {
#pragma unroll
    for (int o = 16; o > 0; o >>= 1) v += __shfl_xor_sync(0xffffffffu, v, o);
    return v;
}

struct pcb_ep { const float *scale, *shift; int act; float slope; };

int pcb_generic_forward(const pcb_conv *c, const void *w, const float *bias, void *y, int y_cstride, const float *msum, cudaStream_t st);
int pcb_generic_dgrad(const pcb_conv *c, const void *dc, int dc_cstride, const void *w_krsc, void *const *dx, const int *dx_cstride,
                      cudaStream_t st);
int pcb_generic_wgrad(const pcb_conv *c, const void *dc, int dc_cstride, float *dw, bool zero_dw, cudaStream_t st);
int pcb_mask_sums(const pcb_conv *c, float *msum, uint8_t *newmask, cudaStream_t st);
bool pcb_tc_eligible(const pcb_conv *c);
size_t pcb_tc_workspace(const pcb_conv *c);
void pcb_tc_weight_layout(const pcb_conv *c, size_t *fwd_elems, size_t *dgrad_elems);
int pcb_tc_weight_prepare(const pcb_conv *c, const float *w_master, void *w_fwd, void *w_dgrad, bool zero_padding, cudaStream_t st);
int pcb_tc_forward_mask_pass(const pcb_conv *c, uint64_t *tapmask, cudaStream_t st);
int pcb_tc_forward_ws(const pcb_conv *c, const void *w_fwd, const float *bias, void *y, int y_cstride, const float *msum,
                      uint64_t *tapmask, bool mask_pass_done, double *bn_sums, const pcb_ep *ep, cudaStream_t st);
bool pcb_tc_fuses_epilogue(const pcb_conv *c);
bool pcb_tc_subpixel(const pcb_conv *c);
int pcb_tc_dgrad(const pcb_conv *c, const void *dc, int dc_cstride, const void *w_dgrad, void *const *dx, const int *dx_cstride,
                 cudaStream_t st, const void *relu_x = nullptr, int relu_cstride = 0);
bool pcb_tc_dgrad_fuses_relu(const pcb_conv *c);
int pcb_tc_wgrad(const pcb_conv *c, const void *dc, int dc_cstride, float *dw, void *workspace, bool zero_dw, cudaStream_t st);
int pcb_tc_read_abort_flag(int *value);
void pcb_tc_routes(const pcb_conv *c, int32_t routes[3]);
struct pcb_smallco_layout { int ktap, koff[2], cout64; long long kf, kd; };
bool pcb_smallco_eligible(const pcb_conv *c);
int pcb_smallco_forward(const pcb_conv *c, const pcb_smallco_layout &L, const void *w_fwd, const float *bias, void *y, int y_cstride, const float *msum,
                        cudaStream_t st);
int pcb_smallco_dgrad(const pcb_conv *c, const pcb_smallco_layout &L, const void *dc, int dc_cstride, const void *w_dgrad, void *const *dx, const int *dx_cstride,
                      cudaStream_t st);
int pcb_smallco_wgrad(const pcb_conv *c, const pcb_smallco_layout &L, const void *dc, int dc_cstride, float *dw, bool zero_dw, cudaStream_t st);
struct K2rPlan {
    bool ok;
    int pu, ps;
    int cu, cs, choff_u, choff_s;
    pcb_conv sub;
    size_t sub_fe, sub_de;
    size_t fwd_extra, dg_extra;
    size_t workspace;
};
K2rPlan pcb_k2r_plan(const pcb_conv *c);
int pcb_k2r_weight_prepare(const pcb_conv *c, const K2rPlan &K, const float *w_master, void *w_fwd_extra, void *w_dg_extra, bool zero_padding,
                           cudaStream_t st);
int pcb_k2r_forward(const pcb_conv *c, const K2rPlan &K, const pcb_smallco_layout &L, const void *w_fwd, const void *w_fwd_extra, const float *bias,
                    void *y, int y_cstride, const float *msum, void *workspace, cudaStream_t st);
int pcb_k2r_dgrad(const pcb_conv *c, const K2rPlan &K, const pcb_smallco_layout &L, const void *dc, int dc_cstride, const void *w_dgrad,
                  const void *w_dg_extra, void *const *dx, const int *dx_cstride, cudaStream_t st);
int pcb_k2r_wgrad(const pcb_conv *c, const K2rPlan &K, const void *dc, int dc_cstride, float *dw, void *workspace, bool zero_dw, cudaStream_t st);
struct StemPlan {
    bool ok;
    pcb_conv sub;
    size_t sub_fe;
    size_t fwd_extra;
    size_t workspace;
};
StemPlan pcb_stem_plan(const pcb_conv *c);
int pcb_stem_weight_prepare(const pcb_conv *c, const StemPlan &K, const float *w_master, void *w_fwd_extra, bool zero_padding, cudaStream_t st);
int pcb_stem_forward(const pcb_conv *c, const StemPlan &K, const void *w_fwd_extra, const float *bias, void *y, int y_cstride,
                     const float *msum, void *workspace, double *bn_sums, const pcb_ep *ep, cudaStream_t st);
int pcb_stem_wgrad(const pcb_conv *c, const StemPlan &K, const void *dc, int dc_cstride, float *dw, void *workspace, bool zero_dw,
                   cudaStream_t st);
bool pcb_dw_eligible(const pcb_conv *c);
int pcb_dw_weight_prepare(const pcb_conv *c, const float *w_master, void *w_t, cudaStream_t st);
int pcb_dw_forward(const pcb_conv *c, const void *w_t, const float *bias, void *y, int y_cstride, const float *msum, double *bn_sums,
                   const pcb_ep *ep, cudaStream_t st);
int pcb_dw_dgrad(const pcb_conv *c, const void *dc, int dc_cstride, const void *w_t, void *dx, int dx_cstride, cudaStream_t st);
int pcb_dw_wgrad(const pcb_conv *c, const void *dc, int dc_cstride, float *dw, bool zero_dw, cudaStream_t st);
```

text_segmentation_image_inpainting_b200/csrc/pcb_ptx.cuh:

```cuda
#pragma once
#include <cuda.h>
#include <cuda_runtime.h>
#include <stdint.h>

namespace ptx {

__device__ __forceinline__ uint32_t smem_u32(const void *p) { return static_cast<uint32_t>(__cvta_generic_to_shared(p)); }

__device__ __forceinline__ bool elect_one() {
    uint32_t pred = 0;
    asm volatile(
        "{\n\t.reg .pred P;\n\telect.sync _|P, 0xffffffff;\n\tselp.b32 %0, 1, 0, P;\n\t}" : "=r"(pred));
    return pred != 0;
}

__device__ __forceinline__ void mbar_init(uint32_t bar, uint32_t count) {
    asm volatile("mbarrier.init.shared::cta.b64 [%0], %1;" ::"r"(bar), "r"(count) : "memory");
}
__device__ __forceinline__ void fence_mbar_init() { asm volatile("fence.mbarrier_init.release.cluster;" ::: "memory"); }
__device__ __forceinline__ void mbar_arrive(uint32_t bar) {
    asm volatile("mbarrier.arrive.shared::cta.b64 _, [%0];" ::"r"(bar) : "memory");
}
__device__ __forceinline__ void mbar_arrive_expect_tx(uint32_t bar, uint32_t bytes) {
    asm volatile("mbarrier.arrive.expect_tx.shared::cta.b64 _, [%0], %1;" ::"r"(bar), "r"(bytes) : "memory");
}
__device__ __forceinline__ bool mbar_try_wait(uint32_t bar, uint32_t parity) {
    uint32_t ok;
    asm volatile(
        "{\n\t.reg .pred P;\n\t"
        "mbarrier.try_wait.parity.shared::cta.b64 P, [%1], %2;\n\t"
        "selp.b32 %0, 1, 0, P;\n\t}"
        : "=r"(ok)
        : "r"(bar), "r"(parity)
        : "memory");
    return ok != 0;
}
__device__ __forceinline__ bool mbar_wait(uint32_t bar, uint32_t parity, int *abort_flag, int code) {
    if (mbar_try_wait(bar, parity)) return true;
    const long long t0 = clock64();
    for (uint32_t it = 1;; ++it) {
        if (mbar_try_wait(bar, parity)) return true;
        if ((it & 63) == 0) {
            if (*reinterpret_cast<volatile int *>(abort_flag) != 0) return false;
            if (clock64() - t0 > 4000000000ll) break;
        }
    }
    atomicCAS(abort_flag, 0, code);
    return false;
}
__device__ __forceinline__ void cp_async_mbar_arrive(uint32_t bar) {
    asm volatile("cp.async.mbarrier.arrive.shared::cta.b64 [%0];" ::"r"(bar) : "memory");
}

__device__ __forceinline__ void cp_async_16(uint32_t dst, const void *src, bool valid) {
    const uint32_t sz = valid ? 16u : 0u;
    asm volatile("cp.async.cg.shared.global [%0], [%1], 16, %2;" ::"r"(dst), "l"(src), "r"(sz) : "memory");
}
__device__ __forceinline__ void cp_async_commit() { asm volatile("cp.async.commit_group;" ::: "memory"); }
template <int N> __device__ __forceinline__ void cp_async_wait() { asm volatile("cp.async.wait_group %0;" ::"n"(N) : "memory"); }

__device__ __forceinline__ void fence_proxy_async_smem() { asm volatile("fence.proxy.async.shared::cta;" ::: "memory"); }

__device__ __forceinline__ void prefetch_tmap(const CUtensorMap *m) {
    asm volatile("prefetch.tensormap [%0];" ::"l"(reinterpret_cast<uint64_t>(m)) : "memory");
}
__device__ __forceinline__ void tma_load_2d(uint32_t dst, const CUtensorMap *m, int c0, int c1, uint32_t bar) {
    asm volatile(
        "cp.async.bulk.tensor.2d.shared::cluster.global.mbarrier::complete_tx::bytes [%0], [%1, {%3, %4}], [%2];"
        ::"r"(dst), "l"(reinterpret_cast<uint64_t>(m)), "r"(bar), "r"(c0), "r"(c1)
        : "memory");
}
__device__ __forceinline__ void tma_load_4d(uint32_t dst, const CUtensorMap *m, int c0, int c1, int c2, int c3, uint32_t bar) {
    asm volatile(
        "cp.async.bulk.tensor.4d.shared::cluster.global.mbarrier::complete_tx::bytes [%0], [%1, {%3, %4, %5, %6}], [%2];"
        ::"r"(dst), "l"(reinterpret_cast<uint64_t>(m)), "r"(bar), "r"(c0), "r"(c1), "r"(c2), "r"(c3)
        : "memory");
}

__device__ __forceinline__ void wgmma_fence() { asm volatile("wgmma.fence.sync.aligned;" ::: "memory"); }
__device__ __forceinline__ void wgmma_commit() { asm volatile("wgmma.commit_group.sync.aligned;" ::: "memory"); }
template <int N> __device__ __forceinline__ void wgmma_wait() { asm volatile("wgmma.wait_group.sync.aligned %0;" ::"n"(N) : "memory"); }
template <int R> __device__ __forceinline__ void wgmma_fence_regs(float (&d)[R]) {
#pragma unroll
    for (int i = 0; i < R; ++i) asm volatile("" : "+f"(d[i])::"memory");
}
template <int TA, int TB> __device__ __forceinline__ void wgmma_m64n32(float (&d)[16], uint64_t a_desc, uint64_t b_desc) {
    asm volatile(
        "{\n\t"
        "wgmma.mma_async.sync.aligned.m64n32k16.f32.bf16.bf16 "
        "{%0, %1, %2, %3, %4, %5, %6, %7, %8, %9, %10, %11, %12, %13, %14, %15}, %16, %17, 1, 1, 1, %18, %19;\n\t"
        "}"
        : "+f"(d[0]), "+f"(d[1]), "+f"(d[2]), "+f"(d[3]), "+f"(d[4]), "+f"(d[5]), "+f"(d[6]), "+f"(d[7]), "+f"(d[8]), "+f"(d[9]), "+f"(d[10]), "+f"(d[11]), "+f"(d[12]), "+f"(d[13]), "+f"(d[14]), "+f"(d[15])
        : "l"(a_desc), "l"(b_desc), "n"(TA), "n"(TB));
}
template <int TA, int TB, int R> __device__ __forceinline__ void wgmma_m64n64(float (&d)[R], uint64_t a_desc, uint64_t b_desc) {
    static_assert(R >= 32, "m64n64 accumulator");
    asm volatile(
        "{\n\t"
        "wgmma.mma_async.sync.aligned.m64n64k16.f32.bf16.bf16 "
        "{%0, %1, %2, %3, %4, %5, %6, %7, %8, %9, %10, %11, %12, %13, %14, %15, %16, %17, %18, %19, %20, %21, %22, %23, %24, %25, %26, %27, %28, %29, %30, %31}, %32, %33, 1, 1, 1, %34, %35;\n\t"
        "}"
        : "+f"(d[0]), "+f"(d[1]), "+f"(d[2]), "+f"(d[3]), "+f"(d[4]), "+f"(d[5]), "+f"(d[6]), "+f"(d[7]), "+f"(d[8]), "+f"(d[9]), "+f"(d[10]), "+f"(d[11]), "+f"(d[12]), "+f"(d[13]), "+f"(d[14]), "+f"(d[15]), "+f"(d[16]), "+f"(d[17]), "+f"(d[18]), "+f"(d[19]), "+f"(d[20]), "+f"(d[21]), "+f"(d[22]), "+f"(d[23]), "+f"(d[24]), "+f"(d[25]), "+f"(d[26]), "+f"(d[27]), "+f"(d[28]), "+f"(d[29]), "+f"(d[30]), "+f"(d[31])
        : "l"(a_desc), "l"(b_desc), "n"(TA), "n"(TB));
}
template <int TA, int TB> __device__ __forceinline__ void wgmma_m64n128(float (&d)[64], uint64_t a_desc, uint64_t b_desc) {
    asm volatile(
        "{\n\t"
        "wgmma.mma_async.sync.aligned.m64n128k16.f32.bf16.bf16 "
        "{%0, %1, %2, %3, %4, %5, %6, %7, %8, %9, %10, %11, %12, %13, %14, %15, %16, %17, %18, %19, %20, %21, %22, %23, %24, %25, %26, %27, %28, %29, %30, %31, %32, %33, %34, %35, %36, %37, %38, %39, %40, %41, %42, %43, %44, %45, %46, %47, %48, %49, %50, %51, %52, %53, %54, %55, %56, %57, %58, %59, %60, %61, %62, %63}, %64, %65, 1, 1, 1, %66, %67;\n\t"
        "}"
        : "+f"(d[0]), "+f"(d[1]), "+f"(d[2]), "+f"(d[3]), "+f"(d[4]), "+f"(d[5]), "+f"(d[6]), "+f"(d[7]), "+f"(d[8]), "+f"(d[9]), "+f"(d[10]), "+f"(d[11]), "+f"(d[12]), "+f"(d[13]), "+f"(d[14]), "+f"(d[15]), "+f"(d[16]), "+f"(d[17]), "+f"(d[18]), "+f"(d[19]), "+f"(d[20]), "+f"(d[21]), "+f"(d[22]), "+f"(d[23]), "+f"(d[24]), "+f"(d[25]), "+f"(d[26]), "+f"(d[27]), "+f"(d[28]), "+f"(d[29]), "+f"(d[30]), "+f"(d[31]), "+f"(d[32]), "+f"(d[33]), "+f"(d[34]), "+f"(d[35]), "+f"(d[36]), "+f"(d[37]), "+f"(d[38]), "+f"(d[39]), "+f"(d[40]), "+f"(d[41]), "+f"(d[42]), "+f"(d[43]), "+f"(d[44]), "+f"(d[45]), "+f"(d[46]), "+f"(d[47]), "+f"(d[48]), "+f"(d[49]), "+f"(d[50]), "+f"(d[51]), "+f"(d[52]), "+f"(d[53]), "+f"(d[54]), "+f"(d[55]), "+f"(d[56]), "+f"(d[57]), "+f"(d[58]), "+f"(d[59]), "+f"(d[60]), "+f"(d[61]), "+f"(d[62]), "+f"(d[63])
        : "l"(a_desc), "l"(b_desc), "n"(TA), "n"(TB));
}
template <int N, int TA, int TB> __device__ __forceinline__ void wgmma_bf16(float (&d)[N / 2], uint64_t a_desc, uint64_t b_desc) {
    if constexpr (N == 32) wgmma_m64n32<TA, TB>(d, a_desc, b_desc);
    else if constexpr (N == 64) wgmma_m64n64<TA, TB>(d, a_desc, b_desc);
    else if constexpr (N == 128) wgmma_m64n128<TA, TB>(d, a_desc, b_desc);
    else {
        static_assert(N == 256 && TB == 0, "wgmma tile width");
        wgmma_m64n128<TA, TB>(*reinterpret_cast<float (*)[64]>(&d[0]), a_desc, b_desc);
        wgmma_m64n128<TA, TB>(*reinterpret_cast<float (*)[64]>(&d[64]), a_desc, b_desc + (16384 >> 4));
    }
}
template <int N> __device__ __forceinline__ void setmaxnreg_inc() { asm volatile("setmaxnreg.inc.sync.aligned.u32 %0;" ::"n"(N)); }
template <int N> __device__ __forceinline__ void setmaxnreg_dec() { asm volatile("setmaxnreg.dec.sync.aligned.u32 %0;" ::"n"(N)); }
__device__ __forceinline__ void named_sync(int id, int threads) { asm volatile("bar.sync %0, %1;" ::"r"(id), "r"(threads) : "memory"); }

__host__ __device__ __forceinline__ uint64_t make_smem_desc(uint32_t smem_addr, uint32_t lbo_bytes, uint32_t sbo_bytes) {
    uint64_t d = 0;
    d |= static_cast<uint64_t>((smem_addr >> 4) & 0x3FFFu);
    d |= static_cast<uint64_t>((lbo_bytes >> 4) & 0x3FFFu) << 16;
    d |= static_cast<uint64_t>((sbo_bytes >> 4) & 0x3FFFu) << 32;
    d |= 1ull << 62;
    return d;
}

}
```

Measured before the change: 1117.

## Replace stem space-to-depth sub-conv with dedicated warp-specialized wgmma fwd and wgrad kernels

The 7x7 stride-2 stem conv no longer goes through the generic tensor-core path on a space-to-depth tensor. It now uses its own forward kernel: the weights stay resident in shared memory, producer warps gather im2row chunks with cp.async, wgmma warps compute, and epilogue warps stage the output. A dedicated weight-gradient kernel is added too, and the space-to-depth channel count shrinks to 16 when the input has 4 or fewer channels, cutting padded work. This aims to remove generic-path overhead and wasted K, at the cost of a large amount of new, more complex and less general code.

```diff
diff --git a/text_segmentation_image_inpainting_b200/build.py b/text_segmentation_image_inpainting_b200/build.py
--- a/text_segmentation_image_inpainting_b200/build.py
+++ b/text_segmentation_image_inpainting_b200/build.py
@@ -10,7 +10,7 @@
 LIB = os.path.join(HERE, "libpconv_b200.so")
 STAMP = os.path.join(HERE, "libpconv_b200.stamp")
 SOURCES = ["api.cu", "conv_tc.cu", "conv_smallco.cu", "conv_k2r.cu", "conv_stem.cu", "conv_generic.cu", "elementwise.cu", "dwconv.cu", "seg_ops.cu", "inpaint_data.cu", "inpaint_loss.cu", "seg_data.cu", "seg_loss.cu"]
-HEADERS = ["pcb_common.cuh", "pcb_ptx.cuh", "pil_data.cuh", os.path.join("..", "..", "include", "pconv_b200.h")]
+HEADERS = ["pcb_common.cuh", "pcb_ptx.cuh", "pcb_tc_epi.cuh", "pil_data.cuh", os.path.join("..", "..", "include", "pconv_b200.h")]
 NVCC_FLAGS = ["-gencode", "arch=compute_90a,code=sm_90a", "-O3", "-std=c++17", "-lineinfo",
               "-Xcompiler", "-fPIC", "-Xcompiler", "-fvisibility=hidden", "--expt-relaxed-constexpr",
               "-cudart", "static"]
diff --git a/text_segmentation_image_inpainting_b200/csrc/conv_stem.cu b/text_segmentation_image_inpainting_b200/csrc/conv_stem.cu
--- a/text_segmentation_image_inpainting_b200/csrc/conv_stem.cu
+++ b/text_segmentation_image_inpainting_b200/csrc/conv_stem.cu
@@ -2,16 +2,16 @@
 
 #include <algorithm>
 
-#include "pcb_common.cuh"
+#include "pcb_tc_epi.cuh"
 
 namespace {
 
-constexpr int S2D_C = 32;
 constexpr int SK = 4;
 
 size_t rup256(size_t v) { return (v + 255) / 256 * 256; }
-size_t s2d_bytes(const pcb_conv *c) { return rup256(static_cast<size_t>(c->n) * (c->h / 2) * (c->w / 2) * S2D_C * sizeof(bf16)); }
-size_t dwsub_bytes(const pcb_conv *c) { return rup256(sizeof(float) * c->cout * SK * SK * S2D_C); }
+int rup64(int v) { return (v + 63) / 64 * 64; }
+size_t s2d_bytes(const pcb_conv *c, int sc) { return rup256(static_cast<size_t>(c->n) * (c->h / 2) * (c->w / 2) * sc * sizeof(bf16)); }
+size_t dwsub_bytes(const pcb_conv *c, int sc) { return rup256(sizeof(float) * c->cout * SK * SK * sc); }
 
 }
 
@@ -24,23 +24,19 @@
     if (p.x_up || p.c > 8 || p.x_cstride != 8 || (p.mask && p.mask_up != 0) || ((c->h | c->w) & 1)) return K;
     if (p.x && (reinterpret_cast<uintptr_t>(p.x) & 15)) return K;
     if (c->ho != c->h / 2 || c->wo != c->w / 2 || c->cout < 32 || (c->cout & 7)) return K;
-    pcb_conv &S = K.sub;
-    S.n = c->n; S.h = c->h / 2; S.w = c->w / 2; S.cin = S2D_C; S.cout = c->cout; S.kh = S.kw = SK; S.stride = 1; S.pad_h = S.pad_w = 2; S.dil = 1;
-    S.groups = 1; S.ho = S.h; S.wo = S.w; S.dtype = PCB_BF16; S.no_guard = c->no_guard; S.nparts = 1;
-    S.parts[0].x = nullptr; S.parts[0].mask = nullptr; S.parts[0].c = S2D_C; S.parts[0].x_cstride = S2D_C;
-    if (!pcb_tc_eligible(&S)) return K;
-    size_t de;
-    pcb_tc_weight_layout(&S, &K.sub_fe, &de);
-    K.sub_fe = (K.sub_fe + 63) / 64 * 64;
-    K.fwd_extra = K.sub_fe + 2 * static_cast<size_t>(c->cout) * SK * SK * S2D_C;
-    K.workspace = s2d_bytes(c) + dwsub_bytes(c) + pcb_tc_workspace(&S);
+    const long long lim = (1ll << 31) - 1, cells = static_cast<long long>(c->n) * c->ho * c->wo;
+    if (cells * rup64(c->cout) > lim || cells * 32 > lim) return K;
+    K.sc = p.c <= 4 ? 16 : 32;
+    const int bn_f = (c->cout % 128 == 0) ? 128 : 64;
+    K.fwd_extra = static_cast<size_t>((c->cout + bn_f - 1) / bn_f * bn_f) * SK * SK * 64 + 2 * static_cast<size_t>(c->cout) * SK * SK * 32;
+    K.workspace = s2d_bytes(c, 32) + dwsub_bytes(c, 32) + rup256(static_cast<size_t>(cells) * sizeof(uint64_t));
     K.ok = true;
     return K;
 }
 
 namespace {
 
-__global__ void s2d_kernel(const bf16 *__restrict__ x, const uint8_t *__restrict__ mask, bf16 *__restrict__ xs, int n, int h, int w) {
+__global__ void s2d_kernel(const bf16 *__restrict__ x, const uint8_t *__restrict__ mask, bf16 *__restrict__ xs, int n, int h, int w, int cc) {
     const int hs = h >> 1, ws = w >> 1;
     const long long total = static_cast<long long>(n) * hs * ws * 2;
     for (long long i = blockIdx.x * static_cast<long long>(blockDim.x) + threadIdx.x; i < total; i += static_cast<long long>(gridDim.x) * blockDim.x) {
@@ -50,81 +46,364 @@
         const long long t = cell / ws;
         const int sy = static_cast<int>(t % hs), img = static_cast<int>(t / hs);
         const long long q = (static_cast<long long>(img) * h + 2 * sy + a) * w + 2 * sx;
-        uint4 v0 = __ldg(reinterpret_cast<const uint4 *>(x + q * 8)), v1 = __ldg(reinterpret_cast<const uint4 *>(x + q * 8 + 8));
-        if (mask) {
-            if (mask[q] == 0) v0 = make_uint4(0u, 0u, 0u, 0u);
-            if (mask[q + 1] == 0) v1 = make_uint4(0u, 0u, 0u, 0u);
-        }
-        uint4 *dst = reinterpret_cast<uint4 *>(xs + cell * S2D_C + a * 16);
-        dst[0] = v0; dst[1] = v1;
-    }
-}
-
-__global__ void stem_weight_kernel(const float *__restrict__ w, float *__restrict__ wsub, int cout, int cin) {
+        const bool k0 = !mask || mask[q] != 0, k1 = !mask || mask[q + 1] != 0;
+        bf16 *dst = xs + cell * 4 * cc + a * 2 * cc;
+        if (cc == 4) {
+            const uint2 z = make_uint2(0u, 0u);
+            const uint2 v0 = k0 ? __ldg(reinterpret_cast<const uint2 *>(x + q * 8)) : z, v1 = k1 ? __ldg(reinterpret_cast<const uint2 *>(x + q * 8 + 8)) : z;
+            *reinterpret_cast<uint4 *>(dst) = make_uint4(v0.x, v0.y, v1.x, v1.y);
+        } else {
+            const uint4 z = make_uint4(0u, 0u, 0u, 0u);
+            reinterpret_cast<uint4 *>(dst)[0] = k0 ? __ldg(reinterpret_cast<const uint4 *>(x + q * 8)) : z;
+            reinterpret_cast<uint4 *>(dst)[1] = k1 ? __ldg(reinterpret_cast<const uint4 *>(x + q * 8 + 8)) : z;
+        }
+    }
+}
+
+struct StemK { int ja, jb, a, b, ch; };
+__host__ __device__ __forceinline__ StemK stem_k(int k, int sc) {
+    const int cc = sc >> 2;
+    StemK r;
+    r.ja = k / (4 * sc); r.jb = (k / sc) & 3; r.a = (k / (2 * cc)) & 1; r.b = (k / cc) & 1; r.ch = k % cc;
+    return r;
+}
+
+__global__ void stem_weight_kernel(const float *__restrict__ w, bf16 *__restrict__ wst, int cout, int rows, int cin, int sc) {
     const int i = blockIdx.x * blockDim.x + threadIdx.x;
-    if (i >= cout * SK * SK * S2D_C) return;
-    const int k = i % S2D_C, jb = (i / S2D_C) % SK, ja = (i / (S2D_C * SK)) % SK, co = i / (S2D_C * SK * SK);
-    const int ch = k & 7, b = (k >> 3) & 1, a = k >> 4;
-    const int ty = 2 * ja + a - 1, tx = 2 * jb + b - 1;
-    wsub[i] = (ty >= 0 && ty < 7 && tx >= 0 && tx < 7 && ch < cin) ? w[((static_cast<long long>(co) * 7 + ty) * 7 + tx) * cin + ch] : 0.f;
-}
-
-__global__ void stem_dw_gather_kernel(const float *__restrict__ dwsub, float *__restrict__ dw, int cout, int cin) {
+    if (i >= rows * SK * SK * sc) return;
+    const int co = i / (SK * SK * sc);
+    const StemK k = stem_k(i % (SK * SK * sc), sc);
+    const int ty = 2 * k.ja + k.a - 1, tx = 2 * k.jb + k.b - 1;
+    const bool in = co < cout && ty >= 0 && ty < 7 && tx >= 0 && tx < 7 && k.ch < cin;
+    wst[i] = __float2bfloat16_rn(in ? w[((static_cast<long long>(co) * 7 + ty) * 7 + tx) * cin + k.ch] : 0.f);
+}
+
+__global__ void stem_dw_gather_kernel(const float *__restrict__ dwsub, float *__restrict__ dw, int cout, int cin, int sc) {
     const int i = blockIdx.x * blockDim.x + threadIdx.x;
     if (i >= cout * 49 * cin) return;
     const int ch = i % cin, tx = (i / cin) % 7, ty = (i / (cin * 7)) % 7, co = i / (cin * 49);
     const int ja = (ty + 1) >> 1, a = (ty + 1) & 1, jb = (tx + 1) >> 1, b = (tx + 1) & 1;
-    dw[i] += dwsub[((static_cast<long long>(co) * SK + ja) * SK + jb) * S2D_C + (a * 2 + b) * 8 + ch];
-}
-
-int run_s2d(const pcb_conv *c, bf16 *xs, cudaStream_t st) {
+    dw[i] += dwsub[static_cast<long long>(co) * SK * SK * sc + (ja * SK + jb) * sc + (a * 2 + b) * (sc >> 2) + ch];
+}
+
+__device__ __forceinline__ void im2row_chunk(const bf16 *xs, int hs, int ws, int sc, bool rv, int img, int oy, int ox, int kidx, uint32_t dst) {
+    const int ja = kidx / (4 * sc), rem = kidx - ja * 4 * sc, jb = rem / sc, ch0 = rem - jb * sc;
+    const int y = oy + ja - 2, x = ox + jb - 2;
+    const bool ok = rv && y >= 0 && y < hs && x >= 0 && x < ws;
+    const bf16 *src = ok ? xs + ((static_cast<long long>(img) * hs + y) * ws + x) * sc + ch0 : xs;
+    ptx::cp_async_16_ca(dst, src, ok);
+}
+
+constexpr int STEM_THREADS = MMA_THREADS + 4 * 32 + EPI_WARPS * 32;
+constexpr int STEM_PROD_THREADS = 128;
+constexpr int STEM_EPI_WARP0 = MMA_WARPS + 4;
+constexpr uint32_t STEM_W_BLOCK = 64 * 128;
+
+struct StemFwdParams {
+    TcParams P;
+    const bf16 *xs, *wst;
+    int hs, ws, sc, nkb, n_tiles, stages;
+};
+
+__global__ void __launch_bounds__(STEM_THREADS, 1) stem_fwd_kernel(const __grid_constant__ StemFwdParams A) {
+    const TcParams &P = A.P;
+    extern __shared__ uint8_t smem_raw[];
+    const uint32_t smem_base = align1024(ptx::smem_u32(smem_raw));
+    uint8_t *smem_gen = smem_raw + (smem_base - ptx::smem_u32(smem_raw));
+    const int S = A.stages, nkb = A.nkb;
+    const uint32_t sW = smem_base, sA = sW + nkb * STEM_W_BLOCK;
+    const uint32_t sBar = sA + S * A_STAGE_BYTES;
+    const uint32_t bar_full = sBar, bar_empty = sBar + 8 * MAX_RING;
+    const uint32_t acc_full = sBar + 16 * MAX_RING, acc_empty = acc_full + 8;
+    const uint32_t s_stat_addr = sBar + TMA_BAR_BYTES;
+    bf16 *acc_stage = reinterpret_cast<bf16 *>(smem_gen + (s_stat_addr + EPI_STAT_SMEM_BYTES - smem_base));
+
+    const int warp = __shfl_sync(0xffffffffu, threadIdx.x >> 5, 0), lane = threadIdx.x & 31;
+    const int n0 = (blockIdx.x % A.n_tiles) * 64;
+    const int tile0 = blockIdx.x / A.n_tiles, tstep = gridDim.x / A.n_tiles;
+    const int m_tiles = (P.m_total + BLOCK_M - 1) / BLOCK_M;
+
+    if (threadIdx.x == 0) {
+        for (int s = 0; s < MAX_RING; ++s) { ptx::mbar_init(bar_full + 8 * s, STEM_PROD_THREADS); ptx::mbar_init(bar_empty + 8 * s, 2); }
+        ptx::mbar_init(acc_full, MMA_WARPS); ptx::mbar_init(acc_empty, EPI_WARPS);
+        ptx::fence_mbar_init();
+    }
+    const int kw = SK * SK * A.sc;
+    for (int i = threadIdx.x; i < nkb * 64 * 8; i += STEM_THREADS) {
+        const int kb = i >> 9, r = (i >> 3) & 63, ch = i & 7;
+        const uint4 v = __ldg(reinterpret_cast<const uint4 *>(A.wst + static_cast<long long>(n0 + r) * kw + kb * 64 + ch * 8));
+        *reinterpret_cast<uint4 *>(smem_gen + kb * STEM_W_BLOCK + r * 128 + ((ch ^ (r & 7)) << 4)) = v;
+    }
+    ptx::fence_proxy_async_smem();
+    __syncthreads();
+
+    if (warp < MMA_WARPS) {
+        const int e = warp, g = warp >> 2;
+        const bool leader = (threadIdx.x & 127) == 0;
+        const uint64_t desc_a0 = ptx::make_smem_desc(sA + g * 64 * 128, 16, 1024);
+        const uint64_t desc_w0 = ptx::make_smem_desc(sW, 16, 1024);
+        int s = 0;
+        uint32_t ph = 0, aph = 1;
+        bool dead = false;
+        for (int mt = tile0; mt < m_tiles && !dead; mt += tstep) {
+            const ConsRows cr = cons_rows<0>(P, mt * BLOCK_M, e, lane);
+            float acc[32];
+            zero_acc(acc);
+            int held = -1;
+            for (int kb = 0; kb < nkb; ++kb) {
+                if (!__all_sync(0xffffffffu, ptx::mbar_wait(bar_full + 8 * s, ph, P.abort_flag, 131))) { dead = true; break; }
+                ptx::fence_proxy_async_smem();
+                const uint64_t da = desc_a0 + static_cast<uint64_t>(s * (A_STAGE_BYTES >> 4));
+                const uint64_t dw = desc_w0 + static_cast<uint64_t>(kb * (STEM_W_BLOCK >> 4));
+                ptx::wgmma_fence();
+#pragma unroll
+                for (int k = 0; k < 4; ++k) ptx::wgmma_bf16<64, 0, 0>(acc, da + 2 * k, dw + 2 * k);
+                ptx::wgmma_commit();
+                ptx::wgmma_wait<1>();
+                if (held >= 0 && leader) ptx::mbar_arrive(bar_empty + 8 * held);
+                held = s;
+                if (++s == S) { s = 0; ph ^= 1; }
+            }
+            ptx::wgmma_wait<0>();
+            ptx::wgmma_fence_regs(acc);
+            if (held >= 0 && leader) ptx::mbar_arrive(bar_empty + 8 * held);
+            if (dead) break;
+            if (!tma_stage_tile<64, 0>(P, acc, acc_stage, acc_full, acc_empty, aph, e, lane, n0, cr, 132)) break;
+        }
+    } else if (warp < STEM_EPI_WARP0) {
+        const int t = threadIdx.x - MMA_THREADS, chunk = t & 7, r0 = t >> 3;
+        const uint32_t sw = static_cast<uint32_t>((chunk ^ (r0 & 7)) << 4);
+        const int plane = A.hs * A.ws;
+        int s = 0;
+        uint32_t ph = 1;
+        bool dead = false;
+        for (int mt = tile0; mt < m_tiles && !dead; mt += tstep) {
+            int img[8], oy[8], ox[8];
+            bool rv[8];
+#pragma unroll
+            for (int i = 0; i < 8; ++i) {
+                const int m = mt * BLOCK_M + r0 + 16 * i;
+                rv[i] = m < P.m_total;
+                const int mm = rv[i] ? m : 0;
+                img[i] = mm / plane;
+                const int rem = mm - img[i] * plane;
+                oy[i] = rem / A.ws; ox[i] = rem - oy[i] * A.ws;
+            }
+            for (int kb = 0; kb < nkb; ++kb) {
+                if (!ptx::mbar_wait(bar_empty + 8 * s, ph, P.abort_flag, 133)) { dead = true; break; }
+                const uint32_t dst = sA + s * A_STAGE_BYTES + r0 * 128 + sw;
+#pragma unroll
+                for (int i = 0; i < 8; ++i) im2row_chunk(A.xs, A.hs, A.ws, A.sc, rv[i], img[i], oy[i], ox[i], kb * 64 + chunk * 8, dst + i * 16 * 128);
+                ptx::cp_async_mbar_arrive(bar_full + 8 * s);
+                ptx::mbar_arrive(bar_full + 8 * s);
+                if (++s == S) { s = 0; ph ^= 1; }
+            }
+        }
+        ptx::cp_async_wait<0>();
+    } else {
+        const int w = warp - STEM_EPI_WARP0;
+        float *s_stat = P.bn_sums != nullptr ? reinterpret_cast<float *>(smem_gen + (s_stat_addr - smem_base)) + w * EPI_STAT_SLICE : nullptr;
+        int stat_n0 = -1;
+        auto origin = [&](int mt, int &m0, int &tn0) { m0 = mt * BLOCK_M; tn0 = n0; };
+        tma_epilogue_warps<64, 0>(P, tile0, tstep, m_tiles, origin, acc_stage, acc_full, acc_empty, s_stat, stat_n0, w, lane, 134);
+        ptx::named_sync(1, EPI_WARPS * 32);
+        if (s_stat != nullptr && stat_n0 >= 0) tc_stats_final<64>(P, s_stat - w * EPI_STAT_SLICE, w, lane, stat_n0);
+    }
+}
+
+constexpr int STEM_WG_THREADS = MMA_THREADS + 4 * 32;
+
+struct StemWgParams {
+    const bf16 *xs, *dc;
+    float *dwsub;
+    int *abort_flag;
+    int hs, ws, sc, cin, cout, dc_cstride, m_total, kb_per_cta, stages;
+};
+
+template <int MB>
+__global__ void __launch_bounds__(STEM_WG_THREADS, 1) stem_wgrad_kernel(const __grid_constant__ StemWgParams W) {
+    constexpr uint32_t BLK = 64 * 128;
+    constexpr uint32_t A_BYTES = 2 * MB * BLK, STAGE = A_BYTES + BLK;
+    extern __shared__ uint8_t smem_raw[];
+    const uint32_t smem_base = align1024(ptx::smem_u32(smem_raw));
+    const int S = W.stages;
+    const uint32_t bar_full = smem_base + S * STAGE, bar_empty = bar_full + 8 * MAX_RING;
+    const int warp = __shfl_sync(0xffffffffu, threadIdx.x >> 5, 0), lane = threadIdx.x & 31;
+    const int n0 = blockIdx.y * 64;
+    const int total_kb = (W.m_total + 63) / 64;
+    const int kb_begin = blockIdx.x * W.kb_per_cta;
+    const int num_kb = max(0, min(total_kb, kb_begin + W.kb_per_cta) - kb_begin);
+
+    if (threadIdx.x == 0) {
+        for (int s = 0; s < MAX_RING; ++s) { ptx::mbar_init(bar_full + 8 * s, STEM_PROD_THREADS); ptx::mbar_init(bar_empty + 8 * s, 2); }
+        ptx::fence_mbar_init();
+    }
+    __syncthreads();
+    if (warp < MMA_WARPS) {
+        const int g = warp >> 2;
+        const bool leader = (threadIdx.x & 127) == 0;
+        const uint64_t desc_a0 = ptx::make_smem_desc(smem_base + g * MB * BLK, BLK, 1024);
+        const uint64_t desc_b0 = ptx::make_smem_desc(smem_base + A_BYTES, BLK, 1024);
+        float acc[MB][32];
+#pragma unroll
+        for (int j = 0; j < MB; ++j) zero_acc(acc[j]);
+        int s = 0, held = -1;
+        uint32_t ph = 0;
+        bool dead = false;
+        for (int it = 0; it < num_kb; ++it) {
+            if (!__all_sync(0xffffffffu, ptx::mbar_wait(bar_full + 8 * s, ph, W.abort_flag, 231))) { dead = true; break; }
+            ptx::fence_proxy_async_smem();
+            const uint64_t da = desc_a0 + static_cast<uint64_t>(s * (STAGE >> 4)), db = desc_b0 + static_cast<uint64_t>(s * (STAGE >> 4));
+            ptx::wgmma_fence();
+#pragma unroll
+            for (int j = 0; j < MB; ++j)
+#pragma unroll
+                for (int k = 0; k < 4; ++k)
+                    ptx::wgmma_m64n64<1, 1>(acc[j], da + j * (BLK >> 4) + 128 * k, db + 128 * k);
+            ptx::wgmma_commit();
+            ptx::wgmma_wait<1>();
+            if (held >= 0 && leader) ptx::mbar_arrive(bar_empty + 8 * held);
+            held = s;
+            if (++s == S) { s = 0; ph ^= 1; }
+        }
+        ptx::wgmma_wait<0>();
+#pragma unroll
+        for (int j = 0; j < MB; ++j) ptx::wgmma_fence_regs(acc[j]);
+        if (held >= 0 && leader) ptx::mbar_arrive(bar_empty + 8 * held);
+        if (!dead && num_kb > 0) {
+            const int kw = SK * SK * W.sc;
+#pragma unroll
+            for (int j = 0; j < MB; ++j)
+#pragma unroll
+                for (int h = 0; h < 2; ++h) {
+                    const int k = (g * MB + j) * 64 + 16 * (warp & 3) + (lane >> 2) + 8 * h;
+                    const StemK q = stem_k(k, W.sc);
+                    const int ty = 2 * q.ja + q.a - 1, tx = 2 * q.jb + q.b - 1;
+                    if (ty < 0 || ty >= 7 || tx < 0 || tx >= 7 || q.ch >= W.cin) continue;
+#pragma unroll
+                    for (int i = 2 * h; i < 32; i += 4)
+#pragma unroll
+                        for (int l = 0; l < 2; ++l) {
+                            const int co = n0 + 8 * (i >> 2) + 2 * (lane & 3) + l;
+                            if (co < W.cout) atomicAdd(W.dwsub + static_cast<long long>(co) * kw + k, acc[j][i + l]);
+                        }
+                }
+        }
+    } else {
+        const int t = threadIdx.x - MMA_THREADS, chunk = t & 7, r0 = t >> 3;
+        const uint32_t sw = static_cast<uint32_t>((chunk ^ (r0 & 7)) << 4);
+        const int plane = W.hs * W.ws;
+        const int co = n0 + chunk * 8;
+        int s = 0;
+        uint32_t ph = 1;
+        for (int it = 0; it < num_kb; ++it) {
+            if (!ptx::mbar_wait(bar_empty + 8 * s, ph, W.abort_flag, 233)) break;
+            const uint32_t dst = smem_base + s * STAGE + r0 * 128 + sw;
+#pragma unroll
+            for (int i = 0; i < 4; ++i) {
+                const int m = (kb_begin + it) * 64 + r0 + 16 * i;
+                const bool rv = m < W.m_total;
+                const int mm = rv ? m : 0, img = mm / plane, rem = mm - img * plane, oy = rem / W.ws, ox = rem - oy * W.ws;
+                const uint32_t d = dst + i * 16 * 128;
+#pragma unroll
+                for (int b = 0; b < 2 * MB; ++b) im2row_chunk(W.xs, W.hs, W.ws, W.sc, rv, img, oy, ox, b * 64 + chunk * 8, d + b * BLK);
+                const bool ok = rv && co < W.cout;
+                ptx::cp_async_16(d + A_BYTES, ok ? W.dc + static_cast<long long>(mm) * W.dc_cstride + co : W.dc, ok);
+            }
+            ptx::cp_async_mbar_arrive(bar_full + 8 * s);
+            ptx::mbar_arrive(bar_full + 8 * s);
+            if (++s == S) { s = 0; ph ^= 1; }
+        }
+        ptx::cp_async_wait<0>();
+    }
+}
+
+int run_s2d(const pcb_conv *c, int sc, bf16 *xs, cudaStream_t st) {
     const pcb_part &p = c->parts[0];
     PCB_CHECK(p.x != nullptr, "space-to-depth stem: null x");
     const long long total = static_cast<long long>(c->n) * (c->h / 2) * (c->w / 2) * 2;
     const int grid = static_cast<int>(std::max<long long>(1, std::min<long long>((total + 255) / 256, 16ll * pcb_num_sms())));
-    s2d_kernel<<<grid, 256, 0, st>>>(static_cast<const bf16 *>(p.x), p.mask, xs, c->n, c->h, c->w);
+    s2d_kernel<<<grid, 256, 0, st>>>(static_cast<const bf16 *>(p.x), p.mask, xs, c->n, c->h, c->w, sc / 4);
     PCB_LAUNCH_CHECK();
     return 0;
 }
 
-}
-
-int pcb_stem_weight_prepare(const pcb_conv *c, const StemPlan &K, const float *w_master, void *w_fwd_extra, bool zero_padding, cudaStream_t st) {
+constexpr size_t STEM_MAX_SMEM = 227 * 1024;
+
+}
+
+int pcb_stem_weight_prepare(const pcb_conv *c, const StemPlan &K, const float *w_master, void *w_fwd_extra, bool, cudaStream_t st) {
     PCB_CHECK(K.ok && w_fwd_extra, "space-to-depth stem: weight prepare on a layer that does not take this path");
-    float *wsub = reinterpret_cast<float *>(static_cast<bf16 *>(w_fwd_extra) + K.sub_fe);
-    const int total = c->cout * SK * SK * S2D_C;
-    stem_weight_kernel<<<(total + 255) / 256, 256, 0, st>>>(w_master, wsub, c->cout, c->cin);
+    const int rows = rup64(c->cout), total = rows * SK * SK * K.sc;
+    stem_weight_kernel<<<(total + 255) / 256, 256, 0, st>>>(w_master, static_cast<bf16 *>(w_fwd_extra), c->cout, rows, c->cin, K.sc);
     PCB_LAUNCH_CHECK();
-    return pcb_tc_weight_prepare(&K.sub, wsub, w_fwd_extra, nullptr, zero_padding, st);
+    return 0;
 }
 
 int pcb_stem_forward(const pcb_conv *c, const StemPlan &K, const void *w_fwd_extra, const float *bias, void *y, int y_cstride,
                      const float *msum, void *workspace, double *bn_sums, const pcb_ep *ep, cudaStream_t st) {
     PCB_CHECK(K.ok && workspace, "space-to-depth stem forward: wrong layer / no workspace");
-    uint8_t *ws = static_cast<uint8_t *>(workspace);
-    bf16 *xs = reinterpret_cast<bf16 *>(ws);
-    if (int rc = run_s2d(c, xs, st)) return rc;
-    pcb_conv sub = K.sub;
-    sub.parts[0].x = xs;
-    uint64_t *sub_ws = reinterpret_cast<uint64_t *>(ws + s2d_bytes(c) + dwsub_bytes(c));
-    if (int rc = pcb_tc_forward_mask_pass(&sub, sub_ws, st)) return rc;
-    return pcb_tc_forward_ws(&sub, w_fwd_extra, bias, y, y_cstride, msum, sub_ws, true, bn_sums, ep, st);
+    PCB_CHECK((reinterpret_cast<uintptr_t>(y) & 15) == 0, "space-to-depth stem forward: y must be 16-byte aligned");
+    int *flag = pcb_tc_abort_flag();
+    PCB_CHECK(flag != nullptr, "cudaMalloc(abort flag) failed");
+    bf16 *xs = static_cast<bf16 *>(workspace);
+    if (int rc = run_s2d(c, K.sc, xs, st)) return rc;
+    StemFwdParams A;
+    memset(&A, 0, sizeof(A));
+    TcParams &P = A.P;
+    P.n = c->n; P.h = P.ho = c->ho; P.w = P.wo = c->wo; P.cout = c->cout; P.m_total = c->n * c->ho * c->wo;
+    P.nparts = 1; P.no_guard = c->no_guard; P.sub = 1; P.fh = c->ho; P.fw = c->wo;
+    P.bias = bias; P.msum = msum; P.y = static_cast<bf16 *>(y); P.y_cstride = y_cstride; P.abort_flag = flag;
+    P.bn_sums = bn_sums; P.bn_c = c->cout;
+    if (ep != nullptr) { P.ep_on = 1; P.ep_scale = ep->scale; P.ep_shift = ep->shift; P.ep_act = ep->act; P.ep_slope = ep->slope; }
+    A.xs = xs; A.wst = static_cast<const bf16 *>(w_fwd_extra);
+    A.hs = c->ho; A.ws = c->wo; A.sc = K.sc; A.nkb = K.sc / 4; A.n_tiles = rup64(c->cout) / 64;
+    const size_t fixed = 1024 + static_cast<size_t>(A.nkb) * STEM_W_BLOCK + TMA_BAR_BYTES + EPI_STAT_SMEM_BYTES + bf16_stage_bytes(64);
+    A.stages = static_cast<int>(std::min<size_t>(MAX_RING, (STEM_MAX_SMEM - fixed) / A_STAGE_BYTES));
+    PCB_CHECK(A.stages >= 2, "space-to-depth stem forward: the ring does not fit");
+    const size_t smem = fixed + static_cast<size_t>(A.stages) * A_STAGE_BYTES;
+    PCB_SMEM_OPT_IN(stem_fwd_kernel, STEM_MAX_SMEM);
+    const int m_tiles = (P.m_total + BLOCK_M - 1) / BLOCK_M;
+    const int per_n = std::max(1, std::min(m_tiles, pcb_num_sms() / A.n_tiles));
+    stem_fwd_kernel<<<per_n * A.n_tiles, STEM_THREADS, smem, st>>>(A);
+    PCB_LAUNCH_CHECK();
+    return 0;
 }
 
 int pcb_stem_wgrad(const pcb_conv *c, const StemPlan &K, const void *dc, int dc_cstride, float *dw, void *workspace, bool zero_dw,
                    cudaStream_t st) {
     PCB_CHECK(K.ok && workspace, "space-to-depth stem wgrad: wrong layer / no workspace");
+    PCB_CHECK((reinterpret_cast<uintptr_t>(dc) & 15) == 0, "space-to-depth stem wgrad: dc must be 16-byte aligned");
+    int *flag = pcb_tc_abort_flag();
+    PCB_CHECK(flag != nullptr, "cudaMalloc(abort flag) failed");
     if (zero_dw) PCB_CUDA(cudaMemsetAsync(dw, 0, sizeof(float) * c->cout * 49 * c->cin, st));
     uint8_t *ws = static_cast<uint8_t *>(workspace);
     bf16 *xs = reinterpret_cast<bf16 *>(ws);
-    float *dwsub = reinterpret_cast<float *>(ws + s2d_bytes(c));
-    void *sub_ws = ws + s2d_bytes(c) + dwsub_bytes(c);
-    if (int rc = run_s2d(c, xs, st)) return rc;
-    pcb_conv sub = K.sub;
-    sub.parts[0].x = xs;
-    if (int rc = pcb_tc_wgrad(&sub, dc, dc_cstride, dwsub, sub_ws, true, st)) return rc;
+    float *dwsub = reinterpret_cast<float *>(ws + s2d_bytes(c, K.sc));
+    if (int rc = run_s2d(c, K.sc, xs, st)) return rc;
+    PCB_CUDA(cudaMemsetAsync(dwsub, 0, sizeof(float) * c->cout * SK * SK * K.sc, st));
+    StemWgParams W;
+    memset(&W, 0, sizeof(W));
+    W.xs = xs; W.dc = static_cast<const bf16 *>(dc); W.dwsub = dwsub; W.abort_flag = flag;
+    W.hs = c->ho; W.ws = c->wo; W.sc = K.sc; W.cin = c->cin; W.cout = c->cout; W.dc_cstride = dc_cstride; W.m_total = c->n * c->ho * c->wo;
+    const size_t stage = static_cast<size_t>(K.sc / 4 + 1) * 64 * 128;
+    W.stages = static_cast<int>(std::min<size_t>(MAX_RING, (STEM_MAX_SMEM - 1024 - 16 * MAX_RING) / stage));
+    const size_t smem = 1024 + W.stages * stage + 16 * MAX_RING;
+    const int co_tiles = rup64(c->cout) / 64;
+    const int total_kb = (W.m_total + 63) / 64;
+    const int ctas = std::max(1, std::min(total_kb, pcb_num_sms() / co_tiles));
+    W.kb_per_cta = (total_kb + ctas - 1) / ctas;
+    dim3 grid((total_kb + W.kb_per_cta - 1) / W.kb_per_cta, co_tiles);
+    if (K.sc == 16) {
+        PCB_SMEM_OPT_IN(stem_wgrad_kernel<2>, STEM_MAX_SMEM);
+        stem_wgrad_kernel<2><<<grid, STEM_WG_THREADS, smem, st>>>(W);
+    } else {
+        PCB_SMEM_OPT_IN(stem_wgrad_kernel<4>, STEM_MAX_SMEM);
+        stem_wgrad_kernel<4><<<grid, STEM_WG_THREADS, smem, st>>>(W);
+    }
+    PCB_LAUNCH_CHECK();
     const int total = c->cout * 49 * c->cin;
-    stem_dw_gather_kernel<<<(total + 255) / 256, 256, 0, st>>>(dwsub, dw, c->cout, c->cin);
+    stem_dw_gather_kernel<<<(total + 255) / 256, 256, 0, st>>>(dwsub, dw, c->cout, c->cin, K.sc);
     PCB_LAUNCH_CHECK();
     return 0;
 }
diff --git a/text_segmentation_image_inpainting_b200/csrc/conv_tc.cu b/text_segmentation_image_inpainting_b200/csrc/conv_tc.cu
--- a/text_segmentation_image_inpainting_b200/csrc/conv_tc.cu
+++ b/text_segmentation_image_inpainting_b200/csrc/conv_tc.cu
@@ -6,77 +6,9 @@
 
 #include "pcb_common.cuh"
 #include "pcb_ptx.cuh"
+#include "pcb_tc_epi.cuh"
 
 namespace {
-
-constexpr int BLOCK_M = 128;
-constexpr int BLOCK_K = 64;
-constexpr int A_STAGE_BYTES = BLOCK_M * 128;
-constexpr int NUM_PRODUCER_THREADS = 128;
-constexpr int TC_MAX_PARTS = 2;
-constexpr int MMA_WARPS = 8;
-constexpr int MMA_THREADS = MMA_WARPS * 32;
-constexpr int acc_pitch(int block_n) { return block_n + 4; }
-constexpr int acc_stage_bytes(int block_n) { return BLOCK_M * acc_pitch(block_n) * 4; }
-
-inline int rup(int v, int m) { return (v + m - 1) / m * m; }
-
-struct TcPart {
-    const bf16 *x;
-    const uint64_t *tapmask;
-    const uint8_t *mask;
-    bf16 *dx;
-    int c, c8, kext, koff, choff, cstride, xup, mup, dx_cstride;
-};
-
-struct TcParams {
-    int n, h, w, cin, cout, kh, kw, stride, pad_h, pad_w, dil, ho, wo;
-    int m_total;
-    int nparts, no_guard, rowpack;
-    int ncols;
-    int ring_a, ring_b;
-    int ktap;
-    TcPart parts[TC_MAX_PARTS];
-    const float *bias; const float *msum; bf16 *y; int y_cstride;
-    const bf16 *dc; int dc_cstride, dc_c8, dc_kext;
-    const bf16 *relu_x; int relu_cstride;
-    int *abort_flag;
-    int box_w, box_h, box_n, stages, use_fix;
-    int wk_base, wk_row, wk_col;
-    int sub, py, px, fh, fw;
-    double *bn_sums;
-    int bn_c;
-    const float *ep_scale, *ep_shift;
-    int ep_on, ep_act;
-    float ep_slope;
-};
-
-constexpr int STAT_SLICE = 256;
-constexpr int STAT_SMEM_BYTES = MMA_WARPS * STAT_SLICE * 4 + 16;
-constexpr int EPI_WARPS = 4;
-constexpr int EPI_STAT_SLICE = 512;
-constexpr int EPI_STAT_SQ = EPI_STAT_SLICE / 2;
-constexpr int EPI_STAT_SMEM_BYTES = EPI_WARPS * EPI_STAT_SLICE * 4;
-constexpr int bf16_pitch(int block_n) { return block_n + 8; }
-constexpr int bf16_stage_bytes(int block_n) { return BLOCK_M * bf16_pitch(block_n) * 2; }
-
-__device__ __forceinline__ float warp_transpose_sum16(float (&v)[16], int lane) {
-#pragma unroll
-    for (int i = 0; i < 16; ++i) v[i] += __shfl_xor_sync(0xffffffffu, v[i], 16);
-#pragma unroll
-    for (int off = 8, n = 16; off >= 1; off >>= 1, n >>= 1) {
-        const bool upper = (lane & off) != 0;
-#pragma unroll
-        for (int i = 0; i < 8; ++i) {
-            if (i < (n >> 1)) {
-                const float send = upper ? v[i] : v[i + (n >> 1)];
-                const float keep = upper ? v[i + (n >> 1)] : v[i];
-                v[i] = keep + __shfl_xor_sync(0xffffffffu, send, off);
-            }
-        }
-    }
-    return v[0];
-}
 
 __device__ __forceinline__ float warp_transpose_sum(float (&v)[32], int lane) {
 #pragma unroll
@@ -94,53 +26,12 @@
     return v[0];
 }
 
-__device__ __forceinline__ uint32_t align1024(uint32_t a) { return (a + 1023u) & ~1023u; }
-
 __device__ __forceinline__ void load_acc32(const float *src, uint32_t (&r)[32]) {
 #pragma unroll
     for (int j = 0; j < 8; ++j) {
         const uint4 v = reinterpret_cast<const uint4 *>(src)[j];
         r[4 * j] = v.x; r[4 * j + 1] = v.y; r[4 * j + 2] = v.z; r[4 * j + 3] = v.w;
     }
-}
-
-struct EpiRow {
-    long long mo;
-    int m;
-    bool rvalid, hole;
-    float inv;
-    float dscale[TC_MAX_PARTS];
-};
-
-template <int MODE>
-__device__ __forceinline__ EpiRow tc_epi_row(const TcParams &P, int m, bool renorm = true) {
-    EpiRow er;
-    er.m = m;
-    er.rvalid = m < P.m_total;
-    er.inv = 0.f;
-    er.hole = false;
-    er.mo = m;
-    int en = 0, eh = 0, ew = 0;
-    if (MODE == 1 && er.rvalid) {
-        en = m / (P.h * P.w); const int rem = m - en * P.h * P.w; eh = rem / P.w; ew = rem - eh * P.w;
-        eh = eh * P.sub + P.py; ew = ew * P.sub + P.px;
-        er.mo = (static_cast<long long>(en) * P.fh + eh) * P.fw + ew;
-    }
-    if (MODE == 0 && er.rvalid && renorm) {
-        const float s = P.msum ? P.msum[er.mo] : 1.f;
-        er.hole = (s == 0.f) && !P.no_guard;
-        er.inv = er.hole ? 0.f : 1.0f / s;
-    }
-#pragma unroll
-    for (int p = 0; p < TC_MAX_PARTS; ++p) {
-        er.dscale[p] = 1.f;
-        if (MODE == 1 && p < P.nparts) {
-            const TcPart &pt = P.parts[p];
-            if (er.rvalid && pt.dx != nullptr && pt.mask != nullptr)
-                er.dscale[p] = pt.mask[(static_cast<long long>(en) * (P.fh >> pt.mup) + (eh >> pt.mup)) * (P.fw >> pt.mup) + (ew >> pt.mup)] ? 1.f : 0.f;
-        }
-    }
-    return er;
 }
 
 template <int BLOCK_N, int MODE>
@@ -228,20 +119,6 @@
 }
 
 template <int BLOCK_N>
-__device__ __forceinline__ void tc_stats_flush(const TcParams &P, float *s_stat, int lane, int n0, int cb, int ce, int sq_off) {
-    __syncwarp();
-    for (int c0 = cb; c0 < ce; c0 += 32) {
-        const int co = n0 + c0 + lane;
-        if (co < P.bn_c) {
-            atomicAdd(P.bn_sums + co, static_cast<double>(s_stat[c0 - cb + lane]));
-            atomicAdd(P.bn_sums + P.bn_c + co, static_cast<double>(s_stat[sq_off + c0 - cb + lane]));
-        }
-        s_stat[c0 - cb + lane] = 0.f; s_stat[sq_off + c0 - cb + lane] = 0.f;
-    }
-    __syncwarp();
-}
-
-template <int BLOCK_N>
 struct EpiRole {
     static constexpr int HN = (BLOCK_N >= 64) ? BLOCK_N / 2 : BLOCK_N;
     int q, half, cb, ce;
@@ -278,28 +155,7 @@
     ptx::named_sync(1 + g, 128);
 }
 
-template <int BLOCK_N>
-__device__ __forceinline__ void tc_stats_final(const TcParams &P, const float *stat_base, int w, int lane, int stat_n0) {
-    for (int col = w * 32 + lane; col < BLOCK_N; col += EPI_WARPS * 32) {
-        const int co = stat_n0 + col;
-        if (co < P.bn_c) {
-            float a = 0.f, q = 0.f;
-#pragma unroll
-            for (int w4 = 0; w4 < EPI_WARPS; ++w4) { a += stat_base[w4 * EPI_STAT_SLICE + col]; q += stat_base[w4 * EPI_STAT_SLICE + EPI_STAT_SQ + col]; }
-            atomicAdd(P.bn_sums + co, static_cast<double>(a));
-            atomicAdd(P.bn_sums + P.bn_c + co, static_cast<double>(q));
-        }
-    }
-}
-
-template <int R> __device__ __forceinline__ void zero_acc(float (&a)[R]) {
-#pragma unroll
-    for (int i = 0; i < R; ++i) a[i] = 0.f;
-}
-
 constexpr int PERSIST_THREADS = 4 * 32 + MMA_THREADS + 32;
-constexpr int MAX_RING = 8;
-
 template <int BLOCK_N, int MODE>
 __global__ void __launch_bounds__(PERSIST_THREADS, 1)
 pconv_tc_persistent_kernel(const __grid_constant__ TcParams P, const __grid_constant__ CUtensorMap tmap_w) {
@@ -547,198 +403,6 @@
     }
 }
 
-
-constexpr int EPI_WARP0 = MMA_WARPS + 4;
-constexpr int TMA_THREADS = (EPI_WARP0 + EPI_WARPS) * 32;
-constexpr int TMA_FIX_THREADS = 96;
-constexpr int TMA_REGS = 128;
-constexpr int TMA_CONSUMER_REGS = 192, TMA_SUPPORT_REGS = 64;
-static_assert(TMA_THREADS == 512 && 2 * 128 * TMA_CONSUMER_REGS + 2 * 128 * TMA_SUPPORT_REGS == TMA_THREADS * TMA_REGS &&
-              TMA_THREADS * TMA_REGS <= 65536, "TMA-fed fwd / dgrad register budget");
-
-constexpr size_t TMA_BAR_BYTES = 24 * MAX_RING + 16;
-
-template <int BLOCK_N, int MODE>
-__device__ __forceinline__ void tc_epilogue_bf16(const TcParams &P, const EpiRow &er, const bf16 *srow, int lane, int n0, float *s_stat) {
-    const bool stats = (MODE == 0) && (s_stat != nullptr);
-#pragma unroll 1
-    for (int c0 = 0; c0 < BLOCK_N; c0 += 32) {
-        const int col = n0 + c0;
-        bf16 *orow = nullptr;
-        int nstore = 0;
-        int xlocal = 0;
-        float scale = 1.f;
-        if (MODE == 0) {
-            if (er.rvalid && col < P.y_cstride) { orow = P.y + er.mo * P.y_cstride + col; nstore = min(32, P.y_cstride - col); }
-        } else {
-#pragma unroll
-            for (int p = 0; p < TC_MAX_PARTS; ++p) {
-                if (p >= P.nparts) break;
-                const TcPart &pt = P.parts[p];
-                const int local = col - pt.koff;
-                if (local >= 0 && local < pt.kext && pt.dx != nullptr && local < pt.c8 && er.rvalid) {
-                    orow = pt.dx + er.mo * pt.dx_cstride + local;
-                    nstore = min(32, pt.c8 - local);
-                    scale = er.dscale[p];
-                    xlocal = local;
-                }
-            }
-        }
-        if (nstore == 0 && !stats) continue;
-        uint4 o[4];
-#pragma unroll
-        for (int j = 0; j < 4; ++j) o[j] = reinterpret_cast<const uint4 *>(srow + c0)[j];
-        if (MODE == 1 && scale != 1.f) {
-            __nv_bfloat162 *ob = reinterpret_cast<__nv_bfloat162 *>(o);
-#pragma unroll
-            for (int j = 0; j < 16; ++j) {
-                const float2 f = __bfloat1622float2(ob[j]);
-                ob[j] = __floats2bfloat162_rn(f.x * scale, f.y * scale);
-            }
-        }
-        if (MODE == 1 && P.relu_x != nullptr && nstore > 0) {
-            const uint4 *xr = reinterpret_cast<const uint4 *>(P.relu_x + er.mo * P.relu_cstride + xlocal);
-#pragma unroll 1
-            for (int j = 0; j < 4; ++j) {
-                if (j * 8 >= nstore) break;
-                const uint4 xv = xr[j];
-                const __nv_bfloat162 *xb = reinterpret_cast<const __nv_bfloat162 *>(&xv);
-                __nv_bfloat162 *ob = reinterpret_cast<__nv_bfloat162 *>(&o[j]);
-#pragma unroll
-                for (int k = 0; k < 4; ++k) {
-                    const float2 xf = __bfloat1622float2(xb[k]);
-                    const __nv_bfloat162 z = __float2bfloat162_rn(0.f);
-                    ob[k] = __halves2bfloat162(xf.x <= 0.f ? z.x : ob[k].x, xf.y <= 0.f ? z.y : ob[k].y);
-                }
-            }
-        }
-        if (nstore > 0) {
-            uint4 *dst = reinterpret_cast<uint4 *>(orow);
-#pragma unroll
-            for (int j = 0; j < 4; ++j)
-                if (j * 8 < nstore) dst[j] = o[j];
-        }
-        if (stats) {
-            const float live = er.rvalid ? 1.f : 0.f;
-            const __nv_bfloat162 *ob = reinterpret_cast<const __nv_bfloat162 *>(srow + c0);
-            float cs = 0.f, cq = 0.f;
-#pragma unroll 1
-            for (int h = 0; h < 2; ++h) {
-                float v[16];
-#pragma unroll
-                for (int j = 0; j < 8; ++j) {
-                    const float2 f = __bfloat1622float2(ob[8 * h + j]);
-                    v[2 * j] = f.x * live; v[2 * j + 1] = f.y * live;
-                }
-                const float s = warp_transpose_sum16(v, lane);
-#pragma unroll
-                for (int j = 0; j < 8; ++j) {
-                    const float2 f = __bfloat1622float2(ob[8 * h + j]);
-                    const float a = f.x * live, b = f.y * live;
-                    v[2 * j] = a * a; v[2 * j + 1] = b * b;
-                }
-                const float q = warp_transpose_sum16(v, lane);
-                if ((lane >> 4) == h) { cs = s; cq = q; }
-            }
-            s_stat[c0 + lane] += cs;
-            s_stat[EPI_STAT_SQ + c0 + lane] += cq;
-        }
-    }
-}
-
-template <int BLOCK_N, int MODE, typename TileFn>
-__device__ __forceinline__ void tma_epilogue_warps(const TcParams &P, int tile0, int tstep, int num_tiles, TileFn tile_origin,
-                                                   const bf16 *stage, uint32_t acc_full, uint32_t acc_empty, float *s_stat,
-                                                   int &stat_n0, int w, int lane, int code) {
-    const int row = w * 32 + lane;
-    if (s_stat) {
-        for (int i = lane; i < EPI_STAT_SLICE; i += 32) s_stat[i] = 0.f;
-        __syncwarp();
-    }
-    uint32_t ph = 0;
-    for (int tile = tile0; tile < num_tiles; tile += tstep) {
-        int m0, n0;
-        tile_origin(tile, m0, n0);
-        if (n0 < 0) continue;
-        if (s_stat && n0 != stat_n0) {
-            if (stat_n0 >= 0) tc_stats_flush<BLOCK_N>(P, s_stat, lane, stat_n0, 0, BLOCK_N, EPI_STAT_SQ);
-            stat_n0 = n0;
-        }
-        const EpiRow er = tc_epi_row<MODE>(P, m0 + row, false);
-        if (!__all_sync(0xffffffffu, ptx::mbar_wait(acc_full, ph, P.abort_flag, code))) { stat_n0 = -1; return; }
-        ph ^= 1;
-        tc_epilogue_bf16<BLOCK_N, MODE>(P, er, stage + row * bf16_pitch(BLOCK_N), lane, n0, s_stat);
-        __syncwarp();
-        if (lane == 0) ptx::mbar_arrive(acc_empty);
-    }
-}
-
-struct ConsRows {
-    float inv[2];
-    bool hole[2];
-};
-template <int MODE>
-__device__ __forceinline__ ConsRows cons_rows(const TcParams &P, int m0, int e, int lane) {
-    ConsRows cr;
-#pragma unroll
-    for (int h = 0; h < 2; ++h) {
-        cr.inv[h] = 0.f; cr.hole[h] = false;
-        if (MODE == 0) {
-            const EpiRow er = tc_epi_row<0>(P, m0 + 64 * (e >> 2) + 16 * (e & 3) + (lane >> 2) + 8 * h);
-            cr.inv[h] = er.inv; cr.hole[h] = er.hole;
-        }
-    }
-    return cr;
-}
-
-template <int BLOCK_N, int MODE>
-__device__ __forceinline__ void stage_acc_bf16(const TcParams &P, const float (&acc)[BLOCK_N / 2], bf16 *stage, int e, int lane, int n0,
-                                               const ConsRows &cr) {
-    constexpr int PITCH = bf16_pitch(BLOCK_N);
-    const int r0 = 64 * (e >> 2) + 16 * (e & 3) + (lane >> 2), c0 = 2 * (lane & 3);
-    const bool has_bias = (MODE == 0) && (P.bias != nullptr);
-    const bool ep = (MODE == 0) && (P.ep_on != 0);
-    const bool ep_aff = ep && (P.ep_scale != nullptr);
-#pragma unroll
-    for (int j = 0; j < BLOCK_N / 8; ++j) {
-        const int col = n0 + 8 * j + c0;
-        float b0 = 0.f, b1 = 0.f, s0 = 1.f, s1 = 1.f, t0 = 0.f, t1 = 0.f;
-        if (MODE == 0) {
-            const bool in0 = col < P.cout, in1 = col + 1 < P.cout;
-            if (has_bias) { if (in0) b0 = __ldg(P.bias + col); if (in1) b1 = __ldg(P.bias + col + 1); }
-            if (ep_aff) {
-                if (in0) { s0 = __ldg(P.ep_scale + col); t0 = __ldg(P.ep_shift + col); }
-                if (in1) { s1 = __ldg(P.ep_scale + col + 1); t1 = __ldg(P.ep_shift + col + 1); }
-            }
-        }
-#pragma unroll
-        for (int h = 0; h < 2; ++h) {
-            float a = acc[4 * j + 2 * h], b = acc[4 * j + 2 * h + 1];
-            if (MODE == 0) {
-                a = cr.hole[h] ? 0.f : fmaf(a, cr.inv[h], b0);
-                b = cr.hole[h] ? 0.f : fmaf(b, cr.inv[h], b1);
-                if (ep) {
-                    a = apply_act(fmaf(a, s0, t0), P.ep_act, P.ep_slope);
-                    b = apply_act(fmaf(b, s1, t1), P.ep_act, P.ep_slope);
-                }
-                if (col >= P.cout) a = 0.f;
-                if (col + 1 >= P.cout) b = 0.f;
-            }
-            *reinterpret_cast<__nv_bfloat162 *>(stage + (r0 + 8 * h) * PITCH + 8 * j + c0) = __floats2bfloat162_rn(a, b);
-        }
-    }
-}
-
-template <int BLOCK_N, int MODE>
-__device__ __forceinline__ bool tma_stage_tile(const TcParams &P, const float (&acc)[BLOCK_N / 2], bf16 *stage, uint32_t acc_full,
-                                               uint32_t acc_empty, uint32_t &ph, int e, int lane, int n0, const ConsRows &cr, int code) {
-    if (!__all_sync(0xffffffffu, ptx::mbar_wait(acc_empty, ph, P.abort_flag, code))) return false;
-    ph ^= 1;
-    stage_acc_bf16<BLOCK_N, MODE>(P, acc, stage, e, lane, n0, cr);
-    __syncwarp();
-    if (lane == 0) ptx::mbar_arrive(acc_full);
-    return true;
-}
 
 template <int BLOCK_N, int MODE, bool HALO>
 __global__ void __maxnreg__(TMA_REGS)
@@ -2609,6 +2273,8 @@
     return launch_wgrad<64, 3, 3>(P, tm, c->cout, st);
 }
 
+int *pcb_tc_abort_flag() { return abort_flag_ptr(); }
+
 int pcb_tc_read_abort_flag(int *value) {
     int *flag = abort_flag_ptr();
     PCB_CHECK(flag != nullptr, "no abort flag");
diff --git a/text_segmentation_image_inpainting_b200/csrc/pcb_common.cuh b/text_segmentation_image_inpainting_b200/csrc/pcb_common.cuh
--- a/text_segmentation_image_inpainting_b200/csrc/pcb_common.cuh
+++ b/text_segmentation_image_inpainting_b200/csrc/pcb_common.cuh
@@ -144,6 +144,7 @@
 bool pcb_tc_dgrad_fuses_relu(const pcb_conv *c);
 int pcb_tc_wgrad(const pcb_conv *c, const void *dc, int dc_cstride, float *dw, void *workspace, bool zero_dw, cudaStream_t st);
 int pcb_tc_read_abort_flag(int *value);
+int *pcb_tc_abort_flag();
 void pcb_tc_routes(const pcb_conv *c, int32_t routes[3]);
 struct pcb_smallco_layout { int ktap, koff[2], cout64; long long kf, kd; };
 bool pcb_smallco_eligible(const pcb_conv *c);
@@ -171,8 +172,7 @@
 int pcb_k2r_wgrad(const pcb_conv *c, const K2rPlan &K, const void *dc, int dc_cstride, float *dw, void *workspace, bool zero_dw, cudaStream_t st);
 struct StemPlan {
     bool ok;
-    pcb_conv sub;
-    size_t sub_fe;
+    int sc;
     size_t fwd_extra;
     size_t workspace;
 };
diff --git a/text_segmentation_image_inpainting_b200/csrc/pcb_ptx.cuh b/text_segmentation_image_inpainting_b200/csrc/pcb_ptx.cuh
--- a/text_segmentation_image_inpainting_b200/csrc/pcb_ptx.cuh
+++ b/text_segmentation_image_inpainting_b200/csrc/pcb_ptx.cuh
@@ -55,6 +55,10 @@
 __device__ __forceinline__ void cp_async_16(uint32_t dst, const void *src, bool valid) {
     const uint32_t sz = valid ? 16u : 0u;
     asm volatile("cp.async.cg.shared.global [%0], [%1], 16, %2;" ::"r"(dst), "l"(src), "r"(sz) : "memory");
+}
+__device__ __forceinline__ void cp_async_16_ca(uint32_t dst, const void *src, bool valid) {
+    const uint32_t sz = valid ? 16u : 0u;
+    asm volatile("cp.async.ca.shared.global [%0], [%1], 16, %2;" ::"r"(dst), "l"(src), "r"(sz) : "memory");
 }
 __device__ __forceinline__ void cp_async_commit() { asm volatile("cp.async.commit_group;" ::: "memory"); }
 template <int N> __device__ __forceinline__ void cp_async_wait() { asm volatile("cp.async.wait_group %0;" ::"n"(N) : "memory"); }
diff --git a/text_segmentation_image_inpainting_b200/csrc/pcb_tc_epi.cuh b/text_segmentation_image_inpainting_b200/csrc/pcb_tc_epi.cuh
--- /dev/null
+++ b/text_segmentation_image_inpainting_b200/csrc/pcb_tc_epi.cuh
@@ -0,0 +1,346 @@
+#pragma once
+#include <cuda.h>
+
+#include "pcb_common.cuh"
+#include "pcb_ptx.cuh"
+
+namespace {
+
+constexpr int BLOCK_M = 128;
+constexpr int BLOCK_K = 64;
+constexpr int A_STAGE_BYTES = BLOCK_M * 128;
+constexpr int NUM_PRODUCER_THREADS = 128;
+constexpr int TC_MAX_PARTS = 2;
+constexpr int MMA_WARPS = 8;
+constexpr int MMA_THREADS = MMA_WARPS * 32;
+constexpr int acc_pitch(int block_n) { return block_n + 4; }
+constexpr int acc_stage_bytes(int block_n) { return BLOCK_M * acc_pitch(block_n) * 4; }
+
+inline int rup(int v, int m) { return (v + m - 1) / m * m; }
+
+struct TcPart {
+    const bf16 *x;
+    const uint64_t *tapmask;
+    const uint8_t *mask;
+    bf16 *dx;
+    int c, c8, kext, koff, choff, cstride, xup, mup, dx_cstride;
+};
+
+struct TcParams {
+    int n, h, w, cin, cout, kh, kw, stride, pad_h, pad_w, dil, ho, wo;
+    int m_total;
+    int nparts, no_guard, rowpack;
+    int ncols;
+    int ring_a, ring_b;
+    int ktap;
+    TcPart parts[TC_MAX_PARTS];
+    const float *bias; const float *msum; bf16 *y; int y_cstride;
+    const bf16 *dc; int dc_cstride, dc_c8, dc_kext;
+    const bf16 *relu_x; int relu_cstride;
+    int *abort_flag;
+    int box_w, box_h, box_n, stages, use_fix;
+    int wk_base, wk_row, wk_col;
+    int sub, py, px, fh, fw;
+    double *bn_sums;
+    int bn_c;
+    const float *ep_scale, *ep_shift;
+    int ep_on, ep_act;
+    float ep_slope;
+};
+
+constexpr int STAT_SLICE = 256;
+constexpr int STAT_SMEM_BYTES = MMA_WARPS * STAT_SLICE * 4 + 16;
+constexpr int EPI_WARPS = 4;
+constexpr int EPI_STAT_SLICE = 512;
+constexpr int EPI_STAT_SQ = EPI_STAT_SLICE / 2;
+constexpr int EPI_STAT_SMEM_BYTES = EPI_WARPS * EPI_STAT_SLICE * 4;
+constexpr int bf16_pitch(int block_n) { return block_n + 8; }
+constexpr int bf16_stage_bytes(int block_n) { return BLOCK_M * bf16_pitch(block_n) * 2; }
+
+__device__ __forceinline__ float warp_transpose_sum16(float (&v)[16], int lane) {
+#pragma unroll
+    for (int i = 0; i < 16; ++i) v[i] += __shfl_xor_sync(0xffffffffu, v[i], 16);
+#pragma unroll
+    for (int off = 8, n = 16; off >= 1; off >>= 1, n >>= 1) {
+        const bool upper = (lane & off) != 0;
+#pragma unroll
+        for (int i = 0; i < 8; ++i) {
+            if (i < (n >> 1)) {
+                const float send = upper ? v[i] : v[i + (n >> 1)];
+                const float keep = upper ? v[i + (n >> 1)] : v[i];
+                v[i] = keep + __shfl_xor_sync(0xffffffffu, send, off);
+            }
+        }
+    }
+    return v[0];
+}
+
+__device__ __forceinline__ uint32_t align1024(uint32_t a) { return (a + 1023u) & ~1023u; }
+
+struct EpiRow {
+    long long mo;
+    int m;
+    bool rvalid, hole;
+    float inv;
+    float dscale[TC_MAX_PARTS];
+};
+
+template <int MODE>
+__device__ __forceinline__ EpiRow tc_epi_row(const TcParams &P, int m, bool renorm = true) {
+    EpiRow er;
+    er.m = m;
+    er.rvalid = m < P.m_total;
+    er.inv = 0.f;
+    er.hole = false;
+    er.mo = m;
+    int en = 0, eh = 0, ew = 0;
+    if (MODE == 1 && er.rvalid) {
+        en = m / (P.h * P.w); const int rem = m - en * P.h * P.w; eh = rem / P.w; ew = rem - eh * P.w;
+        eh = eh * P.sub + P.py; ew = ew * P.sub + P.px;
+        er.mo = (static_cast<long long>(en) * P.fh + eh) * P.fw + ew;
+    }
+    if (MODE == 0 && er.rvalid && renorm) {
+        const float s = P.msum ? P.msum[er.mo] : 1.f;
+        er.hole = (s == 0.f) && !P.no_guard;
+        er.inv = er.hole ? 0.f : 1.0f / s;
+    }
+#pragma unroll
+    for (int p = 0; p < TC_MAX_PARTS; ++p) {
+        er.dscale[p] = 1.f;
+        if (MODE == 1 && p < P.nparts) {
+            const TcPart &pt = P.parts[p];
+            if (er.rvalid && pt.dx != nullptr && pt.mask != nullptr)
+                er.dscale[p] = pt.mask[(static_cast<long long>(en) * (P.fh >> pt.mup) + (eh >> pt.mup)) * (P.fw >> pt.mup) + (ew >> pt.mup)] ? 1.f : 0.f;
+        }
+    }
+    return er;
+}
+
+template <int BLOCK_N>
+__device__ __forceinline__ void tc_stats_flush(const TcParams &P, float *s_stat, int lane, int n0, int cb, int ce, int sq_off) {
+    __syncwarp();
+    for (int c0 = cb; c0 < ce; c0 += 32) {
+        const int co = n0 + c0 + lane;
+        if (co < P.bn_c) {
+            atomicAdd(P.bn_sums + co, static_cast<double>(s_stat[c0 - cb + lane]));
+            atomicAdd(P.bn_sums + P.bn_c + co, static_cast<double>(s_stat[sq_off + c0 - cb + lane]));
+        }
+        s_stat[c0 - cb + lane] = 0.f; s_stat[sq_off + c0 - cb + lane] = 0.f;
+    }
+    __syncwarp();
+}
+
+template <int BLOCK_N>
+__device__ __forceinline__ void tc_stats_final(const TcParams &P, const float *stat_base, int w, int lane, int stat_n0) {
+    for (int col = w * 32 + lane; col < BLOCK_N; col += EPI_WARPS * 32) {
+        const int co = stat_n0 + col;
+        if (co < P.bn_c) {
+            float a = 0.f, q = 0.f;
+#pragma unroll
+            for (int w4 = 0; w4 < EPI_WARPS; ++w4) { a += stat_base[w4 * EPI_STAT_SLICE + col]; q += stat_base[w4 * EPI_STAT_SLICE + EPI_STAT_SQ + col]; }
+            atomicAdd(P.bn_sums + co, static_cast<double>(a));
+            atomicAdd(P.bn_sums + P.bn_c + co, static_cast<double>(q));
+        }
+    }
+}
+
+template <int R> __device__ __forceinline__ void zero_acc(float (&a)[R]) {
+#pragma unroll
+    for (int i = 0; i < R; ++i) a[i] = 0.f;
+}
+
+constexpr int MAX_RING = 8;
+
+constexpr int EPI_WARP0 = MMA_WARPS + 4;
+constexpr int TMA_THREADS = (EPI_WARP0 + EPI_WARPS) * 32;
+constexpr int TMA_FIX_THREADS = 96;
+constexpr int TMA_REGS = 128;
+constexpr int TMA_CONSUMER_REGS = 192, TMA_SUPPORT_REGS = 64;
+static_assert(TMA_THREADS == 512 && 2 * 128 * TMA_CONSUMER_REGS + 2 * 128 * TMA_SUPPORT_REGS == TMA_THREADS * TMA_REGS &&
+              TMA_THREADS * TMA_REGS <= 65536, "TMA-fed fwd / dgrad register budget");
+
+constexpr size_t TMA_BAR_BYTES = 24 * MAX_RING + 16;
+
+template <int BLOCK_N, int MODE>
+__device__ __forceinline__ void tc_epilogue_bf16(const TcParams &P, const EpiRow &er, const bf16 *srow, int lane, int n0, float *s_stat) {
+    const bool stats = (MODE == 0) && (s_stat != nullptr);
+#pragma unroll 1
+    for (int c0 = 0; c0 < BLOCK_N; c0 += 32) {
+        const int col = n0 + c0;
+        bf16 *orow = nullptr;
+        int nstore = 0;
+        int xlocal = 0;
+        float scale = 1.f;
+        if (MODE == 0) {
+            if (er.rvalid && col < P.y_cstride) { orow = P.y + er.mo * P.y_cstride + col; nstore = min(32, P.y_cstride - col); }
+        } else {
+#pragma unroll
+            for (int p = 0; p < TC_MAX_PARTS; ++p) {
+                if (p >= P.nparts) break;
+                const TcPart &pt = P.parts[p];
+                const int local = col - pt.koff;
+                if (local >= 0 && local < pt.kext && pt.dx != nullptr && local < pt.c8 && er.rvalid) {
+                    orow = pt.dx + er.mo * pt.dx_cstride + local;
+                    nstore = min(32, pt.c8 - local);
+                    scale = er.dscale[p];
+                    xlocal = local;
+                }
+            }
+        }
+        if (nstore == 0 && !stats) continue;
+        uint4 o[4];
+#pragma unroll
+        for (int j = 0; j < 4; ++j) o[j] = reinterpret_cast<const uint4 *>(srow + c0)[j];
+        if (MODE == 1 && scale != 1.f) {
+            __nv_bfloat162 *ob = reinterpret_cast<__nv_bfloat162 *>(o);
+#pragma unroll
+            for (int j = 0; j < 16; ++j) {
+                const float2 f = __bfloat1622float2(ob[j]);
+                ob[j] = __floats2bfloat162_rn(f.x * scale, f.y * scale);
+            }
+        }
+        if (MODE == 1 && P.relu_x != nullptr && nstore > 0) {
+            const uint4 *xr = reinterpret_cast<const uint4 *>(P.relu_x + er.mo * P.relu_cstride + xlocal);
+#pragma unroll 1
+            for (int j = 0; j < 4; ++j) {
+                if (j * 8 >= nstore) break;
+                const uint4 xv = xr[j];
+                const __nv_bfloat162 *xb = reinterpret_cast<const __nv_bfloat162 *>(&xv);
+                __nv_bfloat162 *ob = reinterpret_cast<__nv_bfloat162 *>(&o[j]);
+#pragma unroll
+                for (int k = 0; k < 4; ++k) {
+                    const float2 xf = __bfloat1622float2(xb[k]);
+                    const __nv_bfloat162 z = __float2bfloat162_rn(0.f);
+                    ob[k] = __halves2bfloat162(xf.x <= 0.f ? z.x : ob[k].x, xf.y <= 0.f ? z.y : ob[k].y);
+                }
+            }
+        }
+        if (nstore > 0) {
+            uint4 *dst = reinterpret_cast<uint4 *>(orow);
+#pragma unroll
+            for (int j = 0; j < 4; ++j)
+                if (j * 8 < nstore) dst[j] = o[j];
+        }
+        if (stats) {
+            const float live = er.rvalid ? 1.f : 0.f;
+            const __nv_bfloat162 *ob = reinterpret_cast<const __nv_bfloat162 *>(srow + c0);
+            float cs = 0.f, cq = 0.f;
+#pragma unroll 1
+            for (int h = 0; h < 2; ++h) {
+                float v[16];
+#pragma unroll
+                for (int j = 0; j < 8; ++j) {
+                    const float2 f = __bfloat1622float2(ob[8 * h + j]);
+                    v[2 * j] = f.x * live; v[2 * j + 1] = f.y * live;
+                }
+                const float s = warp_transpose_sum16(v, lane);
+#pragma unroll
+                for (int j = 0; j < 8; ++j) {
+                    const float2 f = __bfloat1622float2(ob[8 * h + j]);
+                    const float a = f.x * live, b = f.y * live;
+                    v[2 * j] = a * a; v[2 * j + 1] = b * b;
+                }
+                const float q = warp_transpose_sum16(v, lane);
+                if ((lane >> 4) == h) { cs = s; cq = q; }
+            }
+            s_stat[c0 + lane] += cs;
+            s_stat[EPI_STAT_SQ + c0 + lane] += cq;
+        }
+    }
+}
+
+template <int BLOCK_N, int MODE, typename TileFn>
+__device__ __forceinline__ void tma_epilogue_warps(const TcParams &P, int tile0, int tstep, int num_tiles, TileFn tile_origin,
+                                                   const bf16 *stage, uint32_t acc_full, uint32_t acc_empty, float *s_stat,
+                                                   int &stat_n0, int w, int lane, int code) {
+    const int row = w * 32 + lane;
+    if (s_stat) {
+        for (int i = lane; i < EPI_STAT_SLICE; i += 32) s_stat[i] = 0.f;
+        __syncwarp();
+    }
+    uint32_t ph = 0;
+    for (int tile = tile0; tile < num_tiles; tile += tstep) {
+        int m0, n0;
+        tile_origin(tile, m0, n0);
+        if (n0 < 0) continue;
+        if (s_stat && n0 != stat_n0) {
+            if (stat_n0 >= 0) tc_stats_flush<BLOCK_N>(P, s_stat, lane, stat_n0, 0, BLOCK_N, EPI_STAT_SQ);
+            stat_n0 = n0;
+        }
+        const EpiRow er = tc_epi_row<MODE>(P, m0 + row, false);
+        if (!__all_sync(0xffffffffu, ptx::mbar_wait(acc_full, ph, P.abort_flag, code))) { stat_n0 = -1; return; }
+        ph ^= 1;
+        tc_epilogue_bf16<BLOCK_N, MODE>(P, er, stage + row * bf16_pitch(BLOCK_N), lane, n0, s_stat);
+        __syncwarp();
+        if (lane == 0) ptx::mbar_arrive(acc_empty);
+    }
+}
+
+struct ConsRows {
+    float inv[2];
+    bool hole[2];
+};
+template <int MODE>
+__device__ __forceinline__ ConsRows cons_rows(const TcParams &P, int m0, int e, int lane) {
+    ConsRows cr;
+#pragma unroll
+    for (int h = 0; h < 2; ++h) {
+        cr.inv[h] = 0.f; cr.hole[h] = false;
+        if (MODE == 0) {
+            const EpiRow er = tc_epi_row<0>(P, m0 + 64 * (e >> 2) + 16 * (e & 3) + (lane >> 2) + 8 * h);
+            cr.inv[h] = er.inv; cr.hole[h] = er.hole;
+        }
+    }
+    return cr;
+}
+
+template <int BLOCK_N, int MODE>
+__device__ __forceinline__ void stage_acc_bf16(const TcParams &P, const float (&acc)[BLOCK_N / 2], bf16 *stage, int e, int lane, int n0,
+                                               const ConsRows &cr) {
+    constexpr int PITCH = bf16_pitch(BLOCK_N);
+    const int r0 = 64 * (e >> 2) + 16 * (e & 3) + (lane >> 2), c0 = 2 * (lane & 3);
+    const bool has_bias = (MODE == 0) && (P.bias != nullptr);
+    const bool ep = (MODE == 0) && (P.ep_on != 0);
+    const bool ep_aff = ep && (P.ep_scale != nullptr);
+#pragma unroll
+    for (int j = 0; j < BLOCK_N / 8; ++j) {
+        const int col = n0 + 8 * j + c0;
+        float b0 = 0.f, b1 = 0.f, s0 = 1.f, s1 = 1.f, t0 = 0.f, t1 = 0.f;
+        if (MODE == 0) {
+            const bool in0 = col < P.cout, in1 = col + 1 < P.cout;
+            if (has_bias) { if (in0) b0 = __ldg(P.bias + col); if (in1) b1 = __ldg(P.bias + col + 1); }
+            if (ep_aff) {
+                if (in0) { s0 = __ldg(P.ep_scale + col); t0 = __ldg(P.ep_shift + col); }
+                if (in1) { s1 = __ldg(P.ep_scale + col + 1); t1 = __ldg(P.ep_shift + col + 1); }
+            }
+        }
+#pragma unroll
+        for (int h = 0; h < 2; ++h) {
+            float a = acc[4 * j + 2 * h], b = acc[4 * j + 2 * h + 1];
+            if (MODE == 0) {
+                a = cr.hole[h] ? 0.f : fmaf(a, cr.inv[h], b0);
+                b = cr.hole[h] ? 0.f : fmaf(b, cr.inv[h], b1);
+                if (ep) {
+                    a = apply_act(fmaf(a, s0, t0), P.ep_act, P.ep_slope);
+                    b = apply_act(fmaf(b, s1, t1), P.ep_act, P.ep_slope);
+                }
+                if (col >= P.cout) a = 0.f;
+                if (col + 1 >= P.cout) b = 0.f;
+            }
+            *reinterpret_cast<__nv_bfloat162 *>(stage + (r0 + 8 * h) * PITCH + 8 * j + c0) = __floats2bfloat162_rn(a, b);
+        }
+    }
+}
+
+template <int BLOCK_N, int MODE>
+__device__ __forceinline__ bool tma_stage_tile(const TcParams &P, const float (&acc)[BLOCK_N / 2], bf16 *stage, uint32_t acc_full,
+                                               uint32_t acc_empty, uint32_t &ph, int e, int lane, int n0, const ConsRows &cr, int code) {
+    if (!__all_sync(0xffffffffu, ptx::mbar_wait(acc_empty, ph, P.abort_flag, code))) return false;
+    ph ^= 1;
+    stage_acc_bf16<BLOCK_N, MODE>(P, acc, stage, e, lane, n0, cr);
+    __syncwarp();
+    if (lane == 0) ptx::mbar_arrive(acc_full);
+    return true;
+}
+
+}
```

New measurement: 1156 (median of 6 runs). 3.5% higher.
